# przemo199/ray-tracer-challenge-rs

Measured on AMD Instinct MI355X. Metric: Mray/s (primary+secondary) and ms/frame at 1920x1080, higher is better.
Workload: dtype f32; 1 GPU; three_sphere_scene@1920x1080,depth=5,f32; scene=three_sphere_scene, width=1920, height=1080, max_depth=5, out=real, parallelism=framesx1, rays_per_frame=4147200, stream=side, mode=frames

## Files before the change

profiles/jit/three_sphere_direct.hpp:

```cpp
#pragma once
#include "rtc_internal.hpp"
namespace rtc {
namespace jit {
constexpr int kBegin[7] = {0, 3, 6, 6, 6, 6, 6};
constexpr ShapeRec<float> kShapes[7] = {
    {{__builtin_bit_cast(float, 0x3f800000u), __builtin_bit_cast(float, 0x80000000u), __builtin_bit_cast(float, 0x00000000u), __builtin_bit_cast(float, 0x3f000000u), __builtin_bit_cast(float, 0x80000000u), __builtin_bit_cast(float, 0x3f800000u), __builtin_bit_cast(float, 0x80000000u), __builtin_bit_cast(float, 0xbf800000u), __builtin_bit_cast(float, 0x00000000u), __builtin_bit_cast(float, 0x80000000u), __builtin_bit_cast(float, 0x3f800000u), __builtin_bit_cast(float, 0xbf000000u)}, {__builtin_bit_cast(float, 0xbf000000u), __builtin_bit_cast(float, 0x3f800000u), __builtin_bit_cast(float, 0x3f000000u), __builtin_bit_cast(float, 0x3f805bd1u)}, 3, 1, 1, 774, __builtin_bit_cast(float, 0xff800000u), __builtin_bit_cast(float, 0x7f800000u), {__builtin_bit_cast(float, 0xbf000000u), __builtin_bit_cast(float, 0x3f800000u), __builtin_bit_cast(float, 0x3f000000u), __builtin_bit_cast(float, 0x3f800000u), __builtin_bit_cast(float, 0x00000000u), __builtin_bit_cast(float, 0x00000000u), __builtin_bit_cast(float, 0x00000000u), __builtin_bit_cast(float, 0x00000000u), __builtin_bit_cast(float, 0x00000000u), __builtin_bit_cast(float, 0x00000000u), __builtin_bit_cast(float, 0x00000000u), __builtin_bit_cast(float, 0x00000000u)}},
    {{__builtin_bit_cast(float, 0x40000000u), __builtin_bit_cast(float, 0x80000000u), __builtin_bit_cast(float, 0x00000000u), __builtin_bit_cast(float, 0xc0400000u), __builtin_bit_cast(float, 0x80000000u), __builtin_bit_cast(float, 0x40000000u), __builtin_bit_cast(float, 0x80000000u), __builtin_bit_cast(float, 0xbf800000u), __builtin_bit_cast(float, 0x00000000u), __builtin_bit_cast(float, 0x80000000u), __builtin_bit_cast(float, 0x40000000u), __builtin_bit_cast(float, 0x3f800000u)}, {__builtin_bit_cast(float, 0x3fc00000u), __builtin_bit_cast(float, 0x3f000000u), __builtin_bit_cast(float, 0xbf000000u), __builtin_bit_cast(float, 0x3e807612u)}, 4, 1, 2, 1030, __builtin_bit_cast(float, 0xff800000u), __builtin_bit_cast(float, 0x7f800000u), {__builtin_bit_cast(float, 0x3fc00000u), __builtin_bit_cast(float, 0x3f000000u), __builtin_bit_cast(float, 0xbf000000u), __builtin_bit_cast(float, 0x3e800000u), __builtin_bit_cast(float, 0x00000000u), __builtin_bit_cast(float, 0x00000000u), __builtin_bit_cast(float, 0x00000000u), __builtin_bit_cast(float, 0x00000000u), __builtin_bit_cast(float, 0x00000000u), __builtin_bit_cast(float, 0x00000000u), __builtin_bit_cast(float, 0x00000000u), __builtin_bit_cast(float, 0x00000000u)}},
    {{__builtin_bit_cast(float, 0x4041f07cu), __builtin_bit_cast(float, 0x80000000u), __builtin_bit_cast(float, 0x00000000u), __builtin_bit_cast(float, 0x4091745du), __builtin_bit_cast(float, 0x80000000u), __builtin_bit_cast(float, 0x4041f07cu), __builtin_bit_cast(float, 0x80000000u), __builtin_bit_cast(float, 0xbf800000u), __builtin_bit_cast(float, 0x00000000u), __builtin_bit_cast(float, 0x80000000u), __builtin_bit_cast(float, 0x4041f07cu), __builtin_bit_cast(float, 0x4011745du)}, {__builtin_bit_cast(float, 0xbfc00000u), __builtin_bit_cast(float, 0x3ea8f5c3u), __builtin_bit_cast(float, 0xbf400000u), __builtin_bit_cast(float, 0x3de000b9u)}, 5, 1, 3, 1286, __builtin_bit_cast(float, 0xff800000u), __builtin_bit_cast(float, 0x7f800000u), {__builtin_bit_cast(float, 0xbfc00000u), __builtin_bit_cast(float, 0x3ea8f5c3u), __builtin_bit_cast(float, 0xbf400000u), __builtin_bit_cast(float, 0x3ddf06f7u), __builtin_bit_cast(float, 0x00000000u), __builtin_bit_cast(float, 0x00000000u), __builtin_bit_cast(float, 0x00000000u), __builtin_bit_cast(float, 0x00000000u), __builtin_bit_cast(float, 0x00000000u), __builtin_bit_cast(float, 0x00000000u), __builtin_bit_cast(float, 0x00000000u), __builtin_bit_cast(float, 0x00000000u)}},
    {{__builtin_bit_cast(float, 0x3f800000u), __builtin_bit_cast(float, 0x00000000u), __builtin_bit_cast(float, 0x00000000u), __builtin_bit_cast(float, 0x00000000u), __builtin_bit_cast(float, 0x00000000u), __builtin_bit_cast(float, 0x3f800000u), __builtin_bit_cast(float, 0x00000000u), __builtin_bit_cast(float, 0x00000000u), __builtin_bit_cast(float, 0x00000000u), __builtin_bit_cast(float, 0x00000000u), __builtin_bit_cast(float, 0x3f800000u), __builtin_bit_cast(float, 0x00000000u)}, {__builtin_bit_cast(float, 0x00000000u), __builtin_bit_cast(float, 0x00000000u), __builtin_bit_cast(float, 0x00000000u), __builtin_bit_cast(float, 0xbf800000u)}, 0, 1, 0, 2, __builtin_bit_cast(float, 0xff800000u), __builtin_bit_cast(float, 0x7f800000u), {__builtin_bit_cast(float, 0x00000000u), __builtin_bit_cast(float, 0x00000000u), __builtin_bit_cast(float, 0x00000000u), __builtin_bit_cast(float, 0x00000000u), __builtin_bit_cast(float, 0x00000000u), __builtin_bit_cast(float, 0x00000000u), __builtin_bit_cast(float, 0x00000000u), __builtin_bit_cast(float, 0x00000000u), __builtin_bit_cast(float, 0x00000000u), __builtin_bit_cast(float, 0x00000000u), __builtin_bit_cast(float, 0x00000000u), __builtin_bit_cast(float, 0x00000000u)}},
    {{__builtin_bit_cast(float, 0x3f3b3e17u), __builtin_bit_cast(float, 0x80000000u), __builtin_bit_cast(float, 0x3f2e930eu), __builtin_bit_cast(float, 0xc05a37d2u), __builtin_bit_cast(float, 0xbf2e930eu), __builtin_bit_cast(float, 0xb676812fu), __builtin_bit_cast(float, 0x3f3b3e17u), __builtin_bit_cast(float, 0xc06a0d9du), __builtin_bit_cast(float, 0x36281968u), __builtin_bit_cast(float, 0xbf800000u), __builtin_bit_cast(float, 0xb6344c27u), __builtin_bit_cast(float, 0x37615f30u)}, {__builtin_bit_cast(float, 0x00000000u), __builtin_bit_cast(float, 0x00000000u), __builtin_bit_cast(float, 0x00000000u), __builtin_bit_cast(float, 0xbf800000u)}, 1, 1, 0, 258, __builtin_bit_cast(float, 0xff800000u), __builtin_bit_cast(float, 0x7f800000u), {__builtin_bit_cast(float, 0x00000000u), __builtin_bit_cast(float, 0x00000000u), __builtin_bit_cast(float, 0x00000000u), __builtin_bit_cast(float, 0x00000000u), __builtin_bit_cast(float, 0x00000000u), __builtin_bit_cast(float, 0x00000000u), __builtin_bit_cast(float, 0x00000000u), __builtin_bit_cast(float, 0x00000000u), __builtin_bit_cast(float, 0x00000000u), __builtin_bit_cast(float, 0x00000000u), __builtin_bit_cast(float, 0x00000000u), __builtin_bit_cast(float, 0x00000000u)}},
    {{__builtin_bit_cast(float, 0x3f3b3e17u), __builtin_bit_cast(float, 0x80000000u), __builtin_bit_cast(float, 0xbf2e930eu), __builtin_bit_cast(float, 0x405a37d2u), __builtin_bit_cast(float, 0x3f2e930eu), __builtin_bit_cast(float, 0xb676812fu), __builtin_bit_cast(float, 0x3f3b3e17u), __builtin_bit_cast(float, 0xc06a0d9du), __builtin_bit_cast(float, 0xb6281968u), __builtin_bit_cast(float, 0xbf800000u), __builtin_bit_cast(float, 0xb6344c27u), __builtin_bit_cast(float, 0x37615f30u)}, {__builtin_bit_cast(float, 0x00000000u), __builtin_bit_cast(float, 0x00000000u), __builtin_bit_cast(float, 0x00000000u), __builtin_bit_cast(float, 0xbf800000u)}, 2, 1, 0, 514, __builtin_bit_cast(float, 0xff800000u), __builtin_bit_cast(float, 0x7f800000u), {__builtin_bit_cast(float, 0x00000000u), __builtin_bit_cast(float, 0x00000000u), __builtin_bit_cast(float, 0x00000000u), __builtin_bit_cast(float, 0x00000000u), __builtin_bit_cast(float, 0x00000000u), __builtin_bit_cast(float, 0x00000000u), __builtin_bit_cast(float, 0x00000000u), __builtin_bit_cast(float, 0x00000000u), __builtin_bit_cast(float, 0x00000000u), __builtin_bit_cast(float, 0x00000000u), __builtin_bit_cast(float, 0x00000000u), __builtin_bit_cast(float, 0x00000000u)}},
    {}};
constexpr int kNumClusters = 0;
constexpr float kClusterBall[1][4] = {
    {}};
constexpr int kClusterBegin[1] = {0};
constexpr int kClusterMembers[1] = {0};
constexpr int kNumUnclustered = 6;
constexpr int kUnclustered[6] = {0, 1, 2, 3, 4, 5};
constexpr int kNumLights = 1;
constexpr LightRec<float> kLights[2] = {
    {{__builtin_bit_cast(float, 0xc1200000u), __builtin_bit_cast(float, 0x41200000u), __builtin_bit_cast(float, 0xc1200000u)}, {__builtin_bit_cast(float, 0x3f800000u), __builtin_bit_cast(float, 0x3f800000u), __builtin_bit_cast(float, 0x3f800000u)}},
    {}};
constexpr MaterialRec<float> kMaterials[5] = {
    {{__builtin_bit_cast(float, 0x3f800000u), __builtin_bit_cast(float, 0x3f666666u), __builtin_bit_cast(float, 0x3f666666u)}, __builtin_bit_cast(float, 0x3dcccccdu), __builtin_bit_cast(float, 0x3f666666u), __builtin_bit_cast(float, 0x00000000u), __builtin_bit_cast(float, 0x43480000u), __builtin_bit_cast(float, 0x00000000u), __builtin_bit_cast(float, 0x00000000u), __builtin_bit_cast(float, 0x3f800000u), -1, 1},
    {{__builtin_bit_cast(float, 0x3dcccccdu), __builtin_bit_cast(float, 0x3f800000u), __builtin_bit_cast(float, 0x3f000000u)}, __builtin_bit_cast(float, 0x3dcccccdu), __builtin_bit_cast(float, 0x3f333333u), __builtin_bit_cast(float, 0x3e99999au), __builtin_bit_cast(float, 0x43480000u), __builtin_bit_cast(float, 0x00000000u), __builtin_bit_cast(float, 0x00000000u), __builtin_bit_cast(float, 0x3f800000u), -1, 1},
    {{__builtin_bit_cast(float, 0x3dcccccdu), __builtin_bit_cast(float, 0x3f800000u), __builtin_bit_cast(float, 0x3dcccccdu)}, __builtin_bit_cast(float, 0x3dcccccdu), __builtin_bit_cast(float, 0x3f333333u), __builtin_bit_cast(float, 0x3e99999au), __builtin_bit_cast(float, 0x43480000u), __builtin_bit_cast(float, 0x00000000u), __builtin_bit_cast(float, 0x00000000u), __builtin_bit_cast(float, 0x3f800000u), -1, 1},
    {{__builtin_bit_cast(float, 0x3f800000u), __builtin_bit_cast(float, 0x3f4ccccdu), __builtin_bit_cast(float, 0x3dcccccdu)}, __builtin_bit_cast(float, 0x3dcccccdu), __builtin_bit_cast(float, 0x3f333333u), __builtin_bit_cast(float, 0x3e99999au), __builtin_bit_cast(float, 0x43480000u), __builtin_bit_cast(float, 0x00000000u), __builtin_bit_cast(float, 0x00000000u), __builtin_bit_cast(float, 0x3f800000u), -1, 1},
    {}};
constexpr bool kPatterns = false;
constexpr uint32_t kPatternKinds = 0u;
constexpr bool kTransparent = false;
}
}
```

ray-tracer-challenge-rs_amd/csrc/rtc_host.cpp:

```cpp
#include <hip/hip_runtime.h>

#include <algorithm>
#include <array>
#include <chrono>
#include <cmath>
#include <cstdlib>
#include <cstring>
#include <limits>
#include <memory>
#include <string>
#include <vector>

#include "../../include/rtc.h"
#include "flop_model.hpp"
#include "host_math.hpp"
#include "debug_knobs.hpp"
#include "primary_rect.hpp"
#include "rtc_context.hpp"
#include "rtc_internal.hpp"
#include "shape_identity.hpp"
#include "tri_tree.hpp"
#include "instances.hpp"

namespace rtc {

#define RTC_KERNEL_LAUNCHERS                                                                                          \
    template <typename R>                                                                                             \
    hipError_t launch_trace(const LaunchParams<R>& P, bool pool, bool dup, uint32_t grid, size_t dyn_lds,             \
                            hipStream_t stream);                                                                      \
    template <typename R>                                                                                             \
    hipError_t occupancy(bool pool, bool lds, size_t dyn_lds, int* blocks_per_cu);                                    \
    template <typename R>                                                                                             \
    hipError_t launch_trace_rays(const LaunchParams<R>& P, bool dup, uint32_t grid, size_t dyn_lds, const void* rays, \
                                 void* rgb, void* hits, hipStream_t stream);                                          \
    template <typename R>                                                                                             \
    hipError_t occupancy_rays(bool lds, size_t dyn_lds, int* blocks_per_cu);                                          \
    template <typename R>                                                                                             \
    hipError_t launch_trace_ss(const LaunchParams<R>& P, bool pool, bool dup, uint32_t grid, size_t dyn_lds,          \
                               hipStream_t stream);                                                                   \
    template <typename R>                                                                                             \
    hipError_t occupancy_ss(bool pool, bool lds, size_t dyn_lds, int* blocks_per_cu);
RTC_KERNEL_LAUNCHERS
namespace instanced { RTC_KERNEL_LAUNCHERS }
namespace textured { RTC_KERNEL_LAUNCHERS }
namespace area { RTC_KERNEL_LAUNCHERS }
#undef RTC_KERNEL_LAUNCHERS
namespace sp {
template <typename R>
hipError_t launch_trace(const LaunchParams<R>& P, bool pool, bool dup, uint32_t grid, size_t dyn_lds,
                        hipStream_t stream);
}
constexpr uint32_t kKindsSp = (1u << RT_SHAPE_SPHERE) | (1u << RT_SHAPE_PLANE);

template <typename R>
struct Launchers {
    decltype(&launch_trace<R>) launch_trace;
    decltype(&occupancy<R>) occupancy;
    decltype(&launch_trace_rays<R>) launch_trace_rays;
    decltype(&occupancy_rays<R>) occupancy_rays;
    decltype(&launch_trace_ss<R>) launch_trace_ss;
    decltype(&occupancy_ss<R>) occupancy_ss;
};
#define RTC_BUILD(ns)                                                                                    \
    {ns launch_trace<R>, ns occupancy<R>, ns launch_trace_rays<R>, ns occupancy_rays<R>, ns launch_trace_ss<R>, \
     ns occupancy_ss<R>}
template <typename R>
constexpr Launchers<R> kLaunchers[] = {RTC_BUILD(rtc::), RTC_BUILD(instanced::), RTC_BUILD(textured::), RTC_BUILD(area::)};
#undef RTC_BUILD
template <typename R>
const Launchers<R>& launchers(const rt_context* ctx) {
    return kLaunchers<R>[(uint32_t)ctx->kernel_build];
}

hipError_t launch_order_tiles(uint32_t* cost, uint32_t* order, uint32_t n, uint32_t* n_items, float split_per_cost,
                              uint32_t max_split_log2, float urgent_per_cost, uint32_t graded, uint32_t min_split_log2,
                              hipStream_t stream);
template <typename R>
hipError_t launch_debug_shape(const ShapeRec<R>* shapes, int slot, int kind, uint32_t mode, uint32_t world_space,
                              const double* in, uint32_t n, double* out, hipStream_t stream);

namespace {
thread_local std::string g_error;
}

int set_error(int code, const std::string& msg) {
    g_error = msg;
    return code;
}

void bounding_sphere(const rt_shape_desc& d, double out[4]) {
    out[0] = out[1] = out[2] = 0.0;
    out[3] = -1.0;
    double c[3] = {0.0, 0.0, 0.0}, r = 0.0;
    const double lo = d.minimum, hi = d.maximum;
    switch (d.kind) {
        case RT_SHAPE_SPHERE: r = 1.0; break;
        case RT_SHAPE_CUBE: r = std::sqrt(3.0); break;
        case RT_SHAPE_CYLINDER: {
            if (!std::isfinite(lo) || !std::isfinite(hi) || !(lo <= hi)) return;
            const double half = 0.5 * (hi - lo);
            c[1] = 0.5 * (lo + hi);
            r = std::sqrt(1.0 + half * half);
            break;
        }
        case RT_SHAPE_TRIANGLE: {
            double p[3][3];
            for (int q = 0; q < 3; ++q) {
                p[0][q] = d.vertex_1[q];
                p[1][q] = d.vertex_1[q] + d.edge_1[q];
                p[2][q] = d.vertex_1[q] + d.edge_2[q];
            }
            for (int q = 0; q < 3; ++q) c[q] = (p[0][q] + p[1][q] + p[2][q]) / 3.0;
            for (auto& v : p)
                r = std::max(r, std::sqrt((v[0] - c[0]) * (v[0] - c[0]) + (v[1] - c[1]) * (v[1] - c[1]) +
                                          (v[2] - c[2]) * (v[2] - c[2])));
            break;
        }
        default: return;
    }
    hm::M4 inv;
    for (int i = 0; i < 4; ++i)
        for (int j = 0; j < 4; ++j) inv.m[i][j] = d.inverse[4 * i + j];
    const hm::M4 f = hm::inverse(inv);
    double ftf[3][3] = {}, sigma2 = 0.0;
    for (int i = 0; i < 3; ++i)
        for (int j = 0; j < 3; ++j)
            for (int k = 0; k < 3; ++k) ftf[i][j] += f.m[k][i] * f.m[k][j];
    for (auto& row : ftf) sigma2 = std::max(sigma2, std::fabs(row[0]) + std::fabs(row[1]) + std::fabs(row[2]));
    double wc[3];
    for (int i = 0; i < 3; ++i) wc[i] = f.m[i][0] * c[0] + f.m[i][1] * c[1] + f.m[i][2] * c[2] + f.m[i][3];
    const double wr = r * std::sqrt(sigma2);
    const double scale = std::fabs(wc[0]) + std::fabs(wc[1]) + std::fabs(wc[2]) + wr;
    const double pad = 1e-3 * wr + 1e-4 * scale + 1e-4;
    if (!std::isfinite(wc[0]) || !std::isfinite(wc[1]) || !std::isfinite(wc[2]) || !std::isfinite(wr) ||
        wr + pad > 1e18)
        return;
    for (int i = 0; i < 3; ++i) out[i] = wc[i];
    out[3] = wr + pad;
}

bool similar_sphere(const rt_shape_desc& d, double centre[3], double* r2) {
    if (d.kind != RT_SHAPE_SPHERE) return false;
    hm::M4 inv;
    for (int i = 0; i < 4; ++i)
        for (int j = 0; j < 4; ++j) inv.m[i][j] = d.inverse[4 * i + j];
    if (inv.m[3][0] != 0.0 || inv.m[3][1] != 0.0 || inv.m[3][2] != 0.0 || inv.m[3][3] != 1.0) return false;
    const hm::M4 f = hm::inverse(inv);
    double g[3][3] = {};
    for (int i = 0; i < 3; ++i)
        for (int j = 0; j < 3; ++j)
            for (int k = 0; k < 3; ++k) g[i][j] += f.m[k][i] * f.m[k][j];
    const double s2 = (g[0][0] + g[1][1] + g[2][2]) / 3.0;
    if (!(s2 > 0.0) || !std::isfinite(s2)) return false;
    for (int i = 0; i < 3; ++i)
        for (int j = 0; j < 3; ++j)
            if (!(std::fabs(g[i][j] - (i == j ? s2 : 0.0)) <= 1e-9 * s2)) return false;
    for (int i = 0; i < 3; ++i) {
        centre[i] = f.m[i][3];
        if (!std::isfinite(centre[i])) return false;
    }
    *r2 = s2;
    return true;
}

bool axis_aligned_cube(const rt_shape_desc& d, double face_lo[3], double face_hi[3], double eps[3], double sgn[3]) {
    if (d.kind != RT_SHAPE_CUBE) return false;
    const double* m = d.inverse;
    if (m[12] != 0.0 || m[13] != 0.0 || m[14] != 0.0 || m[15] != 1.0) return false;
    double dmax = 0.0;
// ... 550 lines not shown
    uint64_t n_rays = 0;
    uint32_t depth = 0, out_format = RT_OUT_REAL;
    uint32_t shard_index = 0, shard_count = 1;
    void* out_device = nullptr;
    hipStream_t stream = nullptr;
    uint32_t flags = 0;
    bool image_rows = false;
    uint32_t samples = 0;
    uint32_t out_w = 0, out_h = 0;
};

template <typename R>
void set_instance_params(LaunchParams<R>& P, const DeviceWorld<R>& w) {
    const InstanceCounts& c = w.inst_counts;
    P.n_instances = c.instances;
    P.inst_world_begin = c.instances ? c.world_begin : std::numeric_limits<int32_t>::max();
    P.inst = c.instances ? w.inst.get() : nullptr;
    P.inst_shapes = w.inst_shapes.get();
    P.inst_nodes = w.inst_nodes.get();
    P.inst_pos = w.inst_pos.get();
    P.smooth_plain = w.smooth.plain();
    P.smooth_inst = w.smooth.inst();
    P.uv_plain = w.uv.plain();
    P.uv_inst = w.uv.inst();
    P.texels = w.texels;
    P.textures = w.tex_table;
    P.area = w.n_area ? w.area.get() : nullptr;
    P.n_area = w.n_area;
    P.area_samples = w.area_samples;
    P.area_cull = 1u;
}

template <typename R>
int launch(rt_context* ctx, DeviceWorld<R>& w, const LaunchRequest& q) {
    const rt_camera_desc* cam = q.cam;
    const uint32_t depth = q.depth, flags = q.flags, shard_index = q.shard_index, shard_count = q.shard_count;
    hipStream_t stream = q.stream;
    int rc;
    LaunchParams<R> P{};
    P.image_rows = q.image_rows ? 1u : 0u;
    P.scene = w.scene;
    P.tri_nodes = w.n_tri_nodes ? w.tri_nodes.get() : nullptr;
    P.n_tri_nodes = w.n_tri_nodes;
    P.tri_flat_begin = w.tri_flat_begin;
    set_instance_params(P, w);
    if (!ctx->knobs.area_cull) P.area_cull = 0u;
    if (cam) {
        for (int q = 0; q < 12; ++q) P.cam.inv[q] = (R)cam->inverse[q];
        for (int q = 0; q < 3; ++q) P.cam.origin[q] = (R)cam->origin[q];
        P.cam.half_width = (R)cam->half_width;
        P.cam.half_height = (R)cam->half_height;
        P.cam.pixel_size = (R)cam->pixel_size;
        P.ss_grid = q.samples;
        P.width = q.samples ? q.out_w : cam->width;
        P.height = q.samples ? q.out_h : cam->height;
        P.tiles_x = (P.width + RT_TILE_W - 1) / RT_TILE_W;
        P.tile_rows = tile_rows_for(P.height, shard_count, shard_index);
        P.n_tiles = P.tiles_x * P.tile_rows;
        P.tiles_x_magic = div_magic(P.tiles_x, P.n_tiles);
    } else {
        P.rays = q.d_rays;
        P.n_rays = q.n_rays;
        P.n_tiles = (uint32_t)((q.n_rays + kBlock - 1) / kBlock);
    }
    P.out = q.out_device;
    P.out_format = q.out_format;
    P.shard_index = shard_index;
    P.shard_count = shard_count;
    P.max_depth = depth;
    P.tile_counter = ctx->d_tile_counter.get();
    P.counters = ctx->d_counters.get();
    P.error_flag = ctx->d_error.get();
    if (flags & RT_FLAG_GENERATIONS) P.gen_counts = ctx->d_gen_counts.get();
    if (P.n_tiles == 0) return RT_OK;
    if ((rc = order_after_last(ctx, stream))) return rc;
    LaunchShape ls;
    const bool ss = q.samples != 0;
    rc = plan_launch<R>(ctx, w.scene, depth, P.n_tiles, ls, false, q.samples);
    if (rc) return rc;
    const bool dup = ctx->duplicate_shapes > 0;
    hipFunction_t jf = nullptr;
    if constexpr (sizeof(R) == 4) {
        const uint32_t generic_only =
            RT_FLAG_NO_SHADE | RT_FLAG_NO_TRACE | RT_FLAG_GENERATIONS | (ls.pool ? 0u : RT_FLAG_STAMPS);
        const bool instanced = walked_instances(w), smooth = has_smooth(w);
        const bool tree = w.n_tri_nodes > 0 || instanced || smooth || has_textures(w);
        if (tree && ctx->jit.mode != RT_JIT_OFF && ctx->jit.log.empty())
            ctx->jit.log = has_area(w) ? "no per-scene build: the world has area lights, which the generic kernels sample"
                           : has_textures(w) ? "no per-scene build: the world has textures, which the generic kernels sample"
                           : smooth ? "no per-scene build: the world has smooth triangles, whose normals the generic kernels interpolate"
                           : instanced
                               ? "no per-scene build: the world has mesh instances, which the generic kernels walk"
                               : "no per-scene build: the world has a triangle hierarchy, which the generic kernels walk";
        const bool want = cam && !dup && !tree && !(flags & generic_only) &&
                          (ctx->jit.mode == RT_JIT_SYNC || (ctx->jit.mode >= RT_JIT_AUTO && P.n_tiles >= kJitMinTiles));
        if (want) {
            ++ctx->jit.frames;
            LaunchShape lj = ls;
            if (ctx->knobs.lds_world && !ls.pool && w.scene.kind_begin[kNumKinds] <= kJitRecordsMaxShapes &&
                (rc = plan_launch<R>(ctx, w.scene, depth, P.n_tiles, lj, true, q.samples)))
                return rc;
            int waves = 0;
            if ((rc = jit_function(ctx, lj.pool, lj.world_lds != 0, lj.lds, lj.per_cu, &jf,
                                   (flags & RT_FLAG_NO_SKIPS) != 0, &waves, ss)))
                return rc;
            if (jf && waves > 0 && (rc = plan_pool_for<R>(ctx, jf, lj))) return rc;
            if (jf) ls = lj;
        }
    }
    ctx->jit.used = jf != nullptr;
    P.pool_capacity = ls.cap;
    P.pool_lds_capacity = ls.lcap;
    P.pop_batch = ls.batch;
    if (ls.pool && (rc = check_pixel_range(ctx, depth, sizeof(R) == 4))) return rc;
    P.acc_log2 = acc_shift_f32(ctx->bright_hit, ctx->bright_w, depth);
    if (ls.cap > ls.lcap) {
        const size_t per_block = (size_t)8 * (ls.cap - ls.lcap) * sizeof(R);
        if ((rc = ctx->d_spill.reserve((size_t)ls.grid * per_block))) return rc;
        P.spill = ctx->d_spill.get();
        P.spill_blocks = (uint32_t)(ctx->d_spill.capacity() / per_block);
    }
    P.persistent = ls.sched;
    P.flags = flags;
    P.world_lds = ls.world_lds;
    const bool dynamic = ls.pool;
    if (dynamic) {
        const size_t set = (size_t)kTileQueues * kQueueStride;
        P.tile_counter = ctx->d_tile_counter.get() + (ctx->head_set ? set : 0);
        P.next_tile_counter = ctx->d_tile_counter.get() + (ctx->head_set ? 0 : set);
        if (ls.pool && ctx->knobs.tile_order && cam) {
            if ((rc = plan_tile_order<R>(ctx, ss ? ctx->order_ss : ctx->order, P, cam, depth, ls.grid, stream)))
                return rc;
        }
    }
    if (flags & RT_FLAG_STAMPS) {
        if ((rc = ctx->d_stamps.reserve((size_t)2 * ls.grid))) return rc;
        P.stamps = ctx->d_stamps.get();
        ctx->stamp_count = ls.grid;
        if (ls.pool) {
            const size_t items = (size_t)P.n_tiles << kMaxSplitLog2;
            if ((rc = ctx->d_item_log.reserve(1 + 3 * items))) return rc;
            RT_HIP(hipMemsetAsync(ctx->d_item_log.get(), 0, sizeof(uint64_t), stream));
            P.item_log = ctx->d_item_log.get();
        }
    }
    uint32_t kinds = 0;
    for (int k = 0; k < kNumKinds; ++k)
        if (w.scene.kind_begin[k + 1] > w.scene.kind_begin[k]) kinds |= 1u << k;
    const bool sp = sizeof(R) == 4 && ls.pool && ctx->knobs.kind_variants && (kinds & ~kKindsSp) == 0 && !dup && !ss &&
                    ctx->kernel_build == KernelBuild::plain;
    if (flags & RT_FLAG_FAIL_LAUNCH) return set_error(RT_ERR_HIP, "launch refused (RT_FLAG_FAIL_LAUNCH)");
    if constexpr (sizeof(R) == 4) {
        const size_t ns = ctx->jit.shapes.size();
        if (jf && !ls.pool && cam && !ss && ns <= (size_t)kPrimaryRectSlots && (int)ns == w.scene.kind_begin[kNumKinds] &&
            P.width <= kCullCols * kCullCellW && P.height <= kCullRows * kCullCellH) {
            const uint32_t nc = (P.width + kCullCellW - 1) / kCullCellW, nr = (P.height + kCullCellH - 1) / kCullCellH;
            uint32_t flip_cols[kCullCols + 1] = {}, flip_rows[kCullRows + 1] = {};
            auto outside = [&](const uint32_t r[4], uint32_t b) {
                const bool none = r[0] > r[2] || r[1] > r[3];
                const uint32_t c0 = none ? nc : r[0] / kCullCellW, c1 = none ? nc : r[2] / kCullCellW + 1;
                const uint32_t r0 = none ? nr : r[1] / kCullCellH, r1 = none ? nr : r[3] / kCullCellH + 1;
                flip_cols[0] ^= b, flip_cols[c0] ^= b, flip_cols[c1] ^= b;
                flip_rows[0] ^= b, flip_rows[r0] ^= b, flip_rows[r1] ^= b;
            };
            for (size_t s = 0; s < ns; ++s) {
                uint32_t r[4];
                primary_rect(P.cam, P.width, P.height, ctx->jit.shapes[s].bound, r);
                outside(r, 1u << s);
            }
            const ShadowLayout lay(w.scene.kind_begin, (int)ctx->jit.lights.size());
            if (lay.fits() &&(int)ctx->jit.lights.size() == w.scene.n_lights) {
                for (int p = lay.plane0; p < lay.plane0 + lay.planes; ++p) {
                    const ShapeRec<float>& pl = ctx->jit.shapes[p];
                    const float n[3] = {pl.inv[4], pl.inv[5], pl.inv[6]}, h = -pl.inv[7];
                    uint32_t near[4] = {0, 0, P.width - 1, P.height - 1};
                    for (int l = 0; l < lay.lights; ++l) {
                        const float* lp = ctx->jit.lights[l].position;
                        uint32_t sp[4];
                        shadow_near(P.cam, P.width, P.height, n, h, lp, sp);
                        for (int a = 0; a < 2; ++a) {
                            near[a] = sp[a] > near[a] ? sp[a] : near[a];
                            near[a + 2] = sp[a + 2] < near[a + 2] ? sp[a + 2] : near[a + 2];
                        }
                        for (size_t c = 0; c < ns; ++c) {
                            const int bit = lay.pair_bit(l, p, (int)c);
                            if (bit < 0) continue;
                            if ((int)c == p) {
                                if (shadow_self_clear(P.cam, n, h, lp)) flip_cols[0] ^= 1u << bit;
                                continue;
                            }
                            uint32_t r[4];
                            shadow_rect(P.cam, P.width, P.height, n, h, lp, ctx->jit.shapes[c].bound, r);
                            outside(r, 1u << bit);
                        }
                    }
                    auto blocks = [](uint32_t lo, uint32_t hi, uint32_t cell, uint32_t pixels, uint32_t& b0, uint32_t& b1) {
                        b0 = b1 = 0;
                        if (lo > hi) return;
                        b0 = (lo + cell - 1) / cell;
                        b1 = hi + 1 >= pixels ? (pixels + cell - 1) / cell : (hi + 1) / cell;
                        if (b1 < b0) b1 = b0;
                    };
                    const uint32_t nb = 1u << lay.near_bit(p);
                    uint32_t b0, b1;
                    blocks(near[0], near[2], kCullCellW, P.width, b0, b1);
                    flip_cols[b0] ^= nb, flip_cols[b1] ^= nb;
                    blocks(near[1], near[3], kCullCellH, P.height, b0, b1);
                    flip_rows[b0] ^= nb, flip_rows[b1] ^= nb;
                }
            }
            uint32_t acc = 0;
            for (uint32_t i = 0; i < nc; ++i) P.cull_cols[i] = acc ^= flip_cols[i];
            acc = 0;
            for (uint32_t j = 0; j < nr; ++j) P.cull_rows[j] = acc ^= flip_rows[j];
        }
    }
    if (jf) {
        const ShapeRec<R>* sh = P.scene.shapes;
        const MaterialRec<R>* mt = P.scene.materials;
        const PatternRec<R>* pt = P.scene.patterns;
        const LightRec<R>* lt = P.scene.lights;
        void* args[] = {&P, &sh, &mt, &pt, &lt};
        (void)hipGetLastError();
        RT_HIP(hipModuleLaunchKernel(jf, ls.grid, 1, 1, kBlock, 1, 1, (unsigned)ls.lds, stream, args, nullptr));
    } else if (hipError_t e = ss   ? launchers<R>(ctx).launch_trace_ss(P, ls.pool, dup, ls.grid, ls.lds, stream)
                              : sp ? sp::launch_trace<R>(P, ls.pool, dup, ls.grid, ls.lds, stream)
                                   : launchers<R>(ctx).launch_trace(P, ls.pool, dup, ls.grid, ls.lds, stream);
               e != hipSuccess)
        return set_error(RT_ERR_HIP, std::string("launch of the ") + (ss ? "supersampled " : "") +
                                         (ls.pool ? "pool" : "direct") + " kernel (grid " +
                                         std::to_string(ls.grid) + ", dynamic LDS " + std::to_string(ls.lds) +
                                         " B, pool " + std::to_string(ls.lcap) + "/" + std::to_string(ls.cap) +
                                         " rays in LDS): " + hipGetErrorString(e));
    if (dynamic) ctx->head_set ^= 1;
    ctx->smooth_info.ran_smooth = !jf && has_smooth(w) ? 1u : 0u;
    ctx->texture_info.ran_textured = !jf && has_textures(w) ? 1u : 0u;
    ctx->light_info.ran_area = !jf && has_area(w) ? 1u : 0u;
    return RT_OK;
}

template <typename R>
int ray_blocks_per_cu(rt_context* ctx, bool lds_world, size_t lds, int* per_cu) {
    const int key = 8 + (sizeof(R) == 8 ? 1 : 0) + (lds_world ? 2 : 0);
    if (ctx->occ_lds[key] == lds && ctx->occ_blocks[key] > 0) {
        *per_cu = ctx->occ_blocks[key];
        return RT_OK;
    }
    int api = 0;
    RT_HIP(launchers<R>(ctx).occupancy_rays(lds_world, lds, &api));
    *per_cu = cap_by_lds(api, lds);
    ctx->occ_lds[key] = lds;
    ctx->occ_blocks[key] = *per_cu;
    return RT_OK;
}

template <typename R>
int plan_rays(rt_context* ctx, const DevScene<R>& sc, uint32_t depth, uint32_t n_chunks, LaunchShape& ls) {
    ls.pool = false;
    const size_t wb = world_lds_bytes<R>(sc.kind_begin[kNumKinds], sc.n_materials, sc.n_patterns);
    ls.world_lds = (ctx->knobs.lds_world && wb <= kMaxWorldLds) ? (uint32_t)wb : 0;
    ls.lds = ls.world_lds;
    ls.cap = ray_stack_entries(depth);
    ls.lcap = ls.batch = 0;
    ls.sched = kSchedStatic;
    int per_cu = 0, rc;
    if ((rc = ray_blocks_per_cu<R>(ctx, ls.world_lds != 0, ls.lds, &per_cu))) return rc;
    ls.per_cu = std::max(per_cu, 1);
    const uint64_t resident = (uint64_t)ls.per_cu * (uint64_t)ctx->cu_count;
    ls.grid = (uint32_t)std::max<uint64_t>(1, std::min<uint64_t>(n_chunks, resident));
    ls.grid_tiles = n_chunks;
    return RT_OK;
}

template <typename R>
int launch_rays(rt_context* ctx, DeviceWorld<R>& w, const void* d_rays, uint64_t n, const rt_ray_options* o,
                void* d_rgb, void* d_hits, hipStream_t stream) {
    int rc;
    LaunchParams<R> P{};
    P.scene = w.scene;
    P.tri_nodes = w.n_tri_nodes ? w.tri_nodes.get() : nullptr;
    P.n_tri_nodes = w.n_tri_nodes;
    P.tri_flat_begin = w.tri_flat_begin;
    set_instance_params(P, w);
    if (!ctx->knobs.area_cull) P.area_cull = 0u;
    P.n_rays = n;
    P.n_tiles = (uint32_t)((n + kBlock - 1) / kBlock);
    P.max_depth = o->max_depth;
    P.flags = o->flags;
    P.counters = ctx->d_counters.get();
    P.error_flag = ctx->d_error.get();
    if (o->flags & RT_FLAG_GENERATIONS) P.gen_counts = ctx->d_gen_counts.get();
    if ((rc = order_after_last(ctx, stream))) return rc;
    LaunchShape ls;
    if ((rc = plan_rays<R>(ctx, w.scene, o->max_depth, P.n_tiles, ls))) return rc;
    P.pool_capacity = ls.cap;
    P.persistent = ls.sched;
    P.world_lds = ls.world_lds;
    if (ls.cap) {
        const size_t per_block = ray_stack_word(1, ls.cap, 0, 0) * sizeof(R);
        if ((rc = ctx->d_spill.reserve((size_t)ls.grid * per_block))) return rc;
        P.spill = ctx->d_spill.get();
        P.spill_blocks = (uint32_t)std::min<size_t>(ctx->d_spill.capacity() / per_block, 0xFFFFFFFFu);
    }
    ctx->jit.used = false;
    if (o->flags & RT_FLAG_FAIL_LAUNCH) return set_error(RT_ERR_HIP, "launch refused (RT_FLAG_FAIL_LAUNCH)");
    if (hipError_t e = launchers<R>(ctx).launch_trace_rays(P, ctx->duplicate_shapes > 0, ls.grid, ls.lds, d_rays, d_rgb,
                                                           d_hits, stream);
        e != hipSuccess)
// ... 1563 lines not shown
```

ray-tracer-challenge-rs_amd/csrc/rtc_internal.hpp:

```cpp
#pragma once

#include <cstdint>
#ifndef __HIPCC_RTC__
#include <string>
#endif

#include "../../include/rtc.h"

#if defined(__HIP__)
#define RTC_HD __host__ __device__
#else
#define RTC_HD
#endif

namespace rtc {

#ifndef __HIPCC_RTC__
int set_error(int code, const std::string& msg);
#endif

RTC_HD inline uint32_t shard_tile_rows(uint32_t height, uint32_t shards, uint32_t shard) {
    const uint32_t trows = (height + RT_TILE_H - 1) / RT_TILE_H;
    return trows > shard ? (trows - shard + shards - 1) / shards : 0;
}
RTC_HD inline uint32_t shard_image_row(uint32_t strip_row, uint32_t shards, uint32_t shard) {
    return ((strip_row / RT_TILE_H) * shards + shard) * RT_TILE_H + strip_row % RT_TILE_H;
}
RTC_HD inline void shard_of_image_row(uint32_t y, uint32_t shards, uint32_t* shard, uint32_t* strip_row) {
    const uint32_t trow = y / RT_TILE_H;
    *shard = trow % shards;
    *strip_row = (trow / shards) * RT_TILE_H + y % RT_TILE_H;
}

constexpr int kBlock = 256;
constexpr int kWaves = kBlock / 64;
constexpr int kTileSlots = 1;
constexpr uint32_t kPoolBatch = kBlock;
constexpr int kTilePixels = RT_TILE_W * RT_TILE_H;
static_assert(kTilePixels == kBlock, "one pixel per thread per tile");
constexpr int kNumKinds = 6;
constexpr int kNumCounters = 8;
constexpr int kGenSlots = RT_MAX_SUPPORTED_DEPTH + 1;
constexpr int kCounterShards = 256;
constexpr int kTileQueues = 8;
constexpr int kQueueStride = 32;
constexpr uint32_t kItemTileMask = 0xFFFFFu;
constexpr uint32_t kItemPartShift = 20, kItemSplitShift = 26, kItemPartMask = 63u, kItemSplitMask = 7u;
constexpr uint32_t kItemPrioShift = 29;
constexpr uint32_t kMaxSplitLog2 = 6;
constexpr int kOrderBuilds = 8;
constexpr uint32_t kNoItem = 0xFFFFFFFFu;

struct WorkItem {
    uint32_t tile, part, split_log2, prio;
};
RTC_HD inline WorkItem decode_item(uint32_t item, bool packed) {
    if (!packed) return {item, 0u, 0u, 0u};
    return {item & kItemTileMask, (item >> kItemPartShift) & kItemPartMask, (item >> kItemSplitShift) & kItemSplitMask,
            (item >> kItemPrioShift) & 3u};
}
RTC_HD inline uint32_t encode_item(uint32_t tile, uint32_t part, uint32_t split_log2, uint32_t prio) {
    return tile | part << kItemPartShift | split_log2 << kItemSplitShift | prio << kItemPrioShift;
}
RTC_HD inline bool item_seeds(uint32_t tid, const WorkItem& w) { return (tid >> (8u - w.split_log2)) == w.part; }

RTC_HD inline uint64_t spill_word(uint32_t block, uint32_t spill_cap, uint32_t slot, uint32_t lds_cap) {
    return ((uint64_t)block * spill_cap + (slot - lds_cap)) * 8u;
}

RTC_HD inline uint32_t pool_capacity_ss(uint32_t depth, uint32_t batch, uint32_t grid) {
    (void)grid;
    return (uint32_t)kBlock + depth * batch;
}

RTC_HD inline uint32_t ray_stack_entries(uint32_t max_depth) { return max_depth ? max_depth + 1u : 0u; }
RTC_HD inline uint64_t ray_stack_word(uint32_t block, uint32_t entries, uint32_t e, uint32_t tid) {
    return (((uint64_t)block * entries + e) * 256u + tid) * 8u;
}
constexpr uint64_t kMaxRayBatch = 1ull << 31;

constexpr int32_t kErrPoolOverflow = 1;
constexpr int32_t kErrPoolSpin = 2;
constexpr int32_t kErrBoundsSlot = 4;
constexpr int32_t kErrBoundsSpill = 8;
constexpr int32_t kErrBoundsTile = 16;
constexpr int32_t kErrBoundsOut = 32;
constexpr int32_t kErrPeerTimeout = 64;
constexpr int32_t kErrBitsAll[] = {kErrPoolOverflow, kErrPoolSpin, kErrBoundsSlot, kErrBoundsSpill,
                                   kErrBoundsTile, kErrBoundsOut, kErrPeerTimeout};
#ifndef __HIPCC_RTC__
inline std::string device_error_text(int32_t err) {
    std::string m;
    auto add = [&](int32_t bit, const char* what) {
        if (err & bit) m += (m.empty() ? "" : "; ") + std::string(what);
    };
    add(kErrPoolOverflow, "device ray pool overflow: a child beyond the LIFO bound");
    add(kErrPoolSpin, "device ray pool: a lock's spin bound ran out (a starved wave, not an overflow)");
    add(kErrBoundsSlot, "bounds check: pool slot outside the LIFO bound");
    add(kErrBoundsSpill, "bounds check: spill region outside the spill buffer");
    add(kErrBoundsTile, "bounds check: work item tile outside the launch");
    add(kErrBoundsOut, "bounds check: output index outside the canvas");
    add(kErrPeerTimeout, "peer canvas: a shard's flag (or the owner's release) did not arrive within the timeout");
    const int32_t unknown = err & ~(kErrPoolOverflow | kErrPoolSpin | kErrBoundsSlot | kErrBoundsSpill |
                                    kErrBoundsTile | kErrBoundsOut | kErrPeerTimeout);
    if (unknown) m += (m.empty() ? "" : "; ") + std::string("device error bits ") + std::to_string(unknown);
    return m;
}
#endif

constexpr uint64_t kCanvasFlagAlign = 256;
RTC_HD inline uint32_t div_magic(uint32_t d, uint32_t n) {
    if (d < 2 || (uint64_t)n * d >= (1ull << 32)) return 0;
    return (uint32_t)(((1ull << 32) + d - 1) / d);
}
RTC_HD inline uint32_t div_by(uint32_t t, uint32_t d, uint32_t magic) {
    return magic ? (uint32_t)(((uint64_t)t * magic) >> 32) : t / d;
}

RTC_HD inline uint64_t canvas_flag_offset(uint64_t image_bytes) {
    return (image_bytes + kCanvasFlagAlign - 1) / kCanvasFlagAlign * kCanvasFlagAlign;
}
constexpr uint32_t kSchedGrid = 0;
constexpr uint32_t kSchedDynamic = 1;
constexpr uint32_t kSchedStatic = 2;
constexpr size_t kMaxWorldLds = 16 * 1024;

constexpr double kAccScale = 281474976710656.0;
constexpr double kAccInvScale = 1.0 / 281474976710656.0;
template <bool B, typename T, typename F>
struct Choose {
    using type = T;
};
template <typename T, typename F>
struct Choose<false, T, F> {
    using type = F;
};
#ifndef RTC_ACC_I64
template <typename R>
using PoolAcc = typename Choose<sizeof(R) == 4, int32_t, long long>::type;
#else
template <typename R>
using PoolAcc = long long;
#endif
constexpr uint32_t kAccLog2Min = 8, kAccLog2Max = 28;
#ifndef RTC_POOL_META32
using PoolMeta = uint16_t;
#else
using PoolMeta = uint32_t;
#endif
static_assert(RT_MAX_SUPPORTED_DEPTH < 32, "remaining must fit the pool meta's 8 high bits");

constexpr int32_t kShapeClosed = 1;
constexpr int32_t kShapeClassEnd = 2;
constexpr int32_t kShapeSimilar = 4;
constexpr int32_t kShapeAxisAligned = 8;
constexpr int32_t kShapeSmooth = 16;
constexpr int kSmoothReals = 9;
constexpr int32_t kShapeUV = 32;
constexpr int kUVReals = 6;
struct alignas(16) TexRec {
    uint64_t offset;
    uint32_t width, height;
};
static_assert(sizeof(TexRec) == 16);
constexpr int kShapeClassShift = 8;

template <typename R>
struct alignas(16) ShapeRec {
    R inv[12];
    R bound[4];
    int32_t world_index;
    int32_t casts_shadow;
    int32_t material;
    int32_t flags;
    R ymin, ymax;
    R tri[12];
};

template <typename R>
struct alignas(16) MaterialRec {
    R color[3];
    R ambient, diffuse, specular, shininess;
    R reflectiveness, transparency, refractive_index;
    int32_t pattern;
    int32_t casts_shadow;
};

template <typename R>
struct alignas(16) PatternRec {
    R color_a[3];
    R color_b[3];
    R inv[12];
    int32_t kind;
    int32_t sub_a, sub_b;
    int32_t pad;
};

template <typename R>
constexpr size_t world_lds_bytes(size_t ns, size_t nm, size_t np) {
    return ns * sizeof(ShapeRec<R>) + nm * sizeof(MaterialRec<R>) + np * sizeof(PatternRec<R>) +
           (ns + 3) / 4 * 16;
}
static_assert(sizeof(ShapeRec<float>) % 16 == 0 && sizeof(ShapeRec<double>) % 16 == 0);
static_assert(sizeof(MaterialRec<float>) % 16 == 0 && sizeof(MaterialRec<double>) % 16 == 0);
static_assert(sizeof(PatternRec<float>) % 16 == 0 && sizeof(PatternRec<double>) % 16 == 0);

template <typename R>
struct alignas(16) LightRec {
    R position[3];
    R intensity[3];
};

template <typename R>
struct alignas(16) AreaLightRec {
    R corner[3];
    R uvec[3];
    R vvec[3];
    R intensity[3];
    uint32_t usteps, vsteps, jitter, seed;
};
static_assert(sizeof(AreaLightRec<float>) == 64 && sizeof(AreaLightRec<double>) == 112);

template <typename R>
struct CameraRec {
    R inv[12];
    R origin[3];
    R half_width, half_height, pixel_size;
};

template <typename R>
struct alignas(16) TriNode {
    R ball[4];
    int32_t skip, first, count, pad;
};
static_assert(sizeof(TriNode<float>) == 32 && sizeof(TriNode<double>) == 48);

template <typename R>
struct alignas(16) InstRec {
    R inv[12];
    R ball[4];
    int32_t world_base;
    int32_t casts_shadow;
    int32_t material;
    int32_t n_triangles;
    int32_t node_begin, n_nodes;
    int32_t rec_begin;
    int32_t rec_flat;
    int32_t rec_end;
    int32_t pos_begin;
    int32_t expanded;
    int32_t pad;
};
static_assert(sizeof(InstRec<float>) % 16 == 0 && sizeof(InstRec<double>) % 16 == 0);

template <typename Base>
RTC_HD inline int instance_of_world(Base&& base, int n, int w) {
    int lo = 0, hi = n;
    while (hi - lo > 1) {
        const int mid = (lo + hi) >> 1;
        if (base(mid) <= w) lo = mid;
        else hi = mid;
    }
    return lo;
}

template <typename R>
struct DevScene {
    const ShapeRec<R>* shapes;
    const MaterialRec<R>* materials;
    const PatternRec<R>* patterns;
    const LightRec<R>* lights;
    const int32_t* world_slot;
    const ShapeRec<R>* lshapes;
    const MaterialRec<R>* lmats;
    const PatternRec<R>* lpats;
    const int32_t* lworld_slot;
    int32_t kind_begin[kNumKinds + 1];
    int32_t n_materials, n_patterns;
    int32_t n_lights;
    int32_t any_secondary;
    int32_t no_skips;
};

constexpr int kPrimaryRectSlots = 8;
constexpr uint32_t kCullCellW = 16, kCullCellH = 4;
constexpr uint32_t kCullCols = 128, kCullRows = 512;

constexpr int kShadowRectSlots = 6;
constexpr int kShadowBit0 = kPrimaryRectSlots, kShadowBits = 32 - kPrimaryRectSlots;
struct ShadowLayout {
    int planes, casters, lights, plane0;
    constexpr ShadowLayout(const int32_t* kb, int n_lights)
        : planes(kb[RT_SHAPE_PLANE + 1] - kb[RT_SHAPE_PLANE]), casters(kb[kNumKinds] - planes), lights(n_lights),
          plane0(kb[RT_SHAPE_PLANE]) {}
    constexpr bool fits() const {
        return planes > 0 && lights > 0 && planes + casters <= kShadowRectSlots &&
               planes + lights * planes * (casters + 1) <= kShadowBits;
    }
    constexpr bool is_plane(int slot) const { return slot >= plane0 && slot < plane0 + planes; }
    constexpr int near_bit(int slot) const { return kShadowBit0 + (slot - plane0); }
    constexpr int pair_bit(int light, int slot, int c) const {
        if (is_plane(c) && c != slot) return -1;
        const int rank = c == slot ? casters : (c < plane0 ? c : c - planes);
        return kShadowBit0 + planes + (light * planes + (slot - plane0)) * (casters + 1) + rank;
    }
};

template <typename R>
struct LaunchParams {
    DevScene<R> scene;
    CameraRec<R> cam;
    const double* rays;
    uint64_t n_rays;
    void* out;
    uint32_t out_format;
    uint32_t width, height;
    uint32_t tiles_x;
    uint32_t tile_rows;
    uint32_t image_rows;
    uint32_t shard_index, shard_count;
    uint32_t n_tiles;
    uint32_t max_depth;
    uint32_t pool_capacity;
    uint32_t pool_lds_capacity;
    uint32_t pop_batch;
    uint32_t acc_log2;
    uint32_t persistent;
    uint32_t flags;
    uint32_t world_lds;
    void* spill;
    uint32_t spill_blocks;
    uint32_t tiles_x_magic;
    unsigned long long* stamps;
    unsigned long long* item_log;
    unsigned long long* tile_counter;
    unsigned long long* next_tile_counter;
    const uint32_t* tile_order;
    const uint32_t* item_count;
    uint32_t* tile_cost;
    unsigned long long* counters;
    unsigned long long* gen_counts;
    int32_t* error_flag;
    uint32_t cull_cols[kCullCols];
    uint32_t cull_rows[kCullRows];
    uint32_t ss_grid;
    uint32_t n_tri_nodes;
    const TriNode<R>* tri_nodes;
    uint32_t tri_flat_begin;
    uint32_t n_instances;
    int32_t inst_world_begin;
    const InstRec<R>* inst;
    const ShapeRec<R>* inst_shapes;
    const TriNode<R>* inst_nodes;
    const int32_t* inst_pos;
    const R* smooth_plain;
    const R* smooth_inst;
    const R* uv_plain;
    const R* uv_inst;
    const uint32_t* texels;
    const TexRec* textures;
    const AreaLightRec<R>* area;
    uint32_t n_area;
    uint32_t area_samples;
    uint32_t area_cull;
};

}
```

ray-tracer-challenge-rs_amd/csrc/rtc_jit.cpp:

```cpp
#include <hip/hip_runtime.h>
#include <hip/hiprtc.h>

#include <algorithm>
#include <array>
#include <atomic>
#include <cmath>
#include <cerrno>
#include <chrono>
#include <condition_variable>
#include <cstdio>
#include <cstdlib>
#include <cstring>
#include <map>
#include <memory>
#include <mutex>
#include <string>
#include <thread>
#include <vector>

#include <dirent.h>
#include <dlfcn.h>
#include <fcntl.h>
#include <spawn.h>
#include <sys/stat.h>
#include <sys/wait.h>
#include <unistd.h>

#include "debug_knobs.hpp"
#include "jit_options.hpp"
#include "rtc_context.hpp"
#include "rtc_jit_cache.hpp"
#include "rtc_jit_sources.inc"

extern char** environ;

namespace rtc {

struct CodeBuild {
    std::atomic<int> state{0};
    jitfile::CodeObject co;
    std::string log;
    double ms = 0;
    bool from_disk = false;
};

namespace {

using jitfile::fnv;

std::string hexf(float v) {
    uint32_t b;
    std::memcpy(&b, &v, 4);
    char buf[48];
    std::snprintf(buf, sizeof buf, "__builtin_bit_cast(float, 0x%08xu)", b);
    return buf;
}

template <size_t N>
std::string floats(const float (&a)[N]) {
    std::string s = "{";
    for (size_t i = 0; i < N; ++i) s += (i ? ", " : "") + hexf(a[i]);
    return s + "}";
}
std::string ball4(const float* a) {
    std::string s = "{";
    for (size_t i = 0; i < 4; ++i) s += (i ? ", " : "") + hexf(a[i]);
    return s + "}";
}

constexpr int kClusterMinShapes = 6;
struct Clusters {
    std::vector<std::array<float, 4>> ball;
    std::vector<int> begin, members, unclustered;
};
Clusters make_clusters(const std::vector<ShapeRec<float>>& sh) {
    Clusters c;
    std::vector<int> bounded;
    for (int i = 0; i < (int)sh.size(); ++i) {
        const float r2 = sh[i].bound[3];
        if (std::isfinite(r2) && r2 >= 0.0f) bounded.push_back(i);
        else c.unclustered.push_back(i);
    }
    std::string knob;
    const char* e = debug_knob("jit_clusters", &knob) ? knob.c_str() : nullptr;
    const int n = (int)bounded.size();
    auto flat = [&]() {
        c.unclustered.insert(c.unclustered.end(), bounded.begin(), bounded.end());
        std::sort(c.unclustered.begin(), c.unclustered.end());
        c.ball.clear();
        c.members.clear();
        c.begin = {0};
        return c;
    };
    const int forced = e ? std::atoi(e) : 0;
    if ((n < kClusterMinShapes && !(forced >= 1 && n >= 2)) || (e && !std::strcmp(e, "0"))) return flat();
    using P3 = std::array<double, 3>;
    auto ctr = [&](int i) { return P3{sh[i].bound[0], sh[i].bound[1], sh[i].bound[2]}; };
    auto rad = [&](int i) { return std::sqrt((double)sh[i].bound[3]); };
    auto d2 = [](const P3& a, const P3& b) {
        return (a[0] - b[0]) * (a[0] - b[0]) + (a[1] - b[1]) * (a[1] - b[1]) + (a[2] - b[2]) * (a[2] - b[2]);
    };
    struct Cl {
        P3 cent;
        double r;
        std::vector<int> m;
    };
    auto kmeans = [&](int k) {
        std::vector<P3> cent{ctr(bounded[0])};
        while ((int)cent.size() < k) {
            int far = bounded[0];
            double best = -1.0;
            for (int i : bounded) {
                double m = 1e300;
                for (const auto& q : cent) m = std::min(m, d2(ctr(i), q));
                if (m > best) best = m, far = i;
            }
            cent.push_back(ctr(far));
        }
        std::vector<int> lab(n, 0);
        for (int it = 0; it < 32; ++it) {
            for (int j = 0; j < n; ++j) {
                double m = 1e300;
                for (int q = 0; q < k; ++q)
                    if (const double v = d2(ctr(bounded[j]), cent[q]); v < m) m = v, lab[j] = q;
            }
            for (int q = 0; q < k; ++q) {
                P3 sum{0, 0, 0};
                int cnt = 0;
                for (int j = 0; j < n; ++j)
                    if (lab[j] == q) {
                        const P3 a = ctr(bounded[j]);
                        for (int t = 0; t < 3; ++t) sum[t] += a[t];
                        ++cnt;
                    }
                if (cnt) cent[q] = {sum[0] / cnt, sum[1] / cnt, sum[2] / cnt};
            }
        }
        std::vector<Cl> out;
        for (int q = 0; q < k; ++q) {
            Cl cl{cent[q], 0.0, {}};
            for (int j = 0; j < n; ++j)
                if (lab[j] == q) {
                    cl.m.push_back(bounded[j]);
                    cl.r = std::max(cl.r, std::sqrt(d2(ctr(bounded[j]), cent[q])) + rad(bounded[j]));
                }
            if (!cl.m.empty()) out.push_back(cl);
        }
        return out;
    };
    P3 mid{0, 0, 0};
    for (int i : bounded)
        for (int t = 0; t < 3; ++t) mid[t] += ctr(i)[t] / n;
    double world = 0.0;
    for (int i : bounded) world = std::max(world, std::sqrt(d2(ctr(i), mid)) + rad(i));
    constexpr double kMemberWeight = 2.0;
    std::string rknob;
    const char* rf = debug_knob("jit_cluster_refine", &rknob) ? rknob.c_str() : nullptr;
    const bool refine = !(rf && !std::strcmp(rf, "0")) && n <= 64;
    auto ball_of = [&](Cl& q) {
        q.cent = {0, 0, 0};
        for (int i : q.m)
            for (int t = 0; t < 3; ++t) q.cent[t] += ctr(i)[t] / (double)q.m.size();
        q.r = 0.0;
        for (int i : q.m) q.r = std::max(q.r, std::sqrt(d2(ctr(i), q.cent)) + rad(i));
    };
    auto term = [&](const Cl& q) { return (double)q.m.size() * q.r * q.r; };
    auto refine_clusters = [&](std::vector<Cl>& cl) {
        for (int guard = 0; guard < 256; ++guard) {
            double best_gain = 1e-9 * world * world;
            int ba = -1, bs = -1, bb = -1;
            for (int a = 0; a < (int)cl.size(); ++a) {
                if (cl[a].m.size() < 2) continue;
                for (int si = 0; si < (int)cl[a].m.size(); ++si)
                    for (int b = 0; b < (int)cl.size(); ++b) {
                        if (b == a) continue;
                        Cl na = cl[a], nb = cl[b];
                        na.m.erase(na.m.begin() + si);
                        nb.m.push_back(cl[a].m[si]);
                        ball_of(na);
                        ball_of(nb);
                        const double gain = term(cl[a]) + term(cl[b]) - term(na) - term(nb);
                        if (gain > best_gain) best_gain = gain, ba = a, bs = si, bb = b;
                    }
            }
            if (ba < 0) break;
            cl[bb].m.push_back(cl[ba].m[bs]);
            cl[ba].m.erase(cl[ba].m.begin() + bs);
            ball_of(cl[ba]);
            ball_of(cl[bb]);
        }
        for (Cl& q : cl) std::sort(q.m.begin(), q.m.end());
    };
    std::vector<Cl> best;
    double best_cost = 0.8 * kMemberWeight * n;
    for (int k = forced == 1 ? 1 : 2; k <= std::min(8, n - 1); ++k) {
        if (forced >= 1 && k != std::min(forced, n - 1)) continue;
        std::vector<Cl> cl = kmeans(k);
        if (refine) refine_clusters(cl);
        double cost = (double)cl.size();
        for (const Cl& q : cl) cost += kMemberWeight * (double)q.m.size() * std::min(1.0, (q.r / world) * (q.r / world));
        if (cost < best_cost || forced >= 1) best_cost = cost, best = std::move(cl);
    }
    if (best.empty()) return flat();
    c.begin.push_back(0);
    for (const Cl& q : best) {
        c.members.insert(c.members.end(), q.m.begin(), q.m.end());
        const double pad = 1e-4 * (q.r + std::fabs(q.cent[0]) + std::fabs(q.cent[1]) + std::fabs(q.cent[2])) + 1e-4;
        c.ball.push_back({(float)q.cent[0], (float)q.cent[1], (float)q.cent[2], (float)((q.r + pad) * (q.r + pad))});
        c.begin.push_back((int)c.members.size());
    }
    return c;
}

std::string scene_header(const std::vector<ShapeRec<float>>& sh, const int32_t begin[kNumKinds + 1],
                         const std::vector<LightRec<float>>& lights, const std::vector<MaterialRec<float>>& mats,
                         bool patterns, uint32_t pattern_kinds, bool transparent) {
    std::string s = "#pragma once\n#include \"rtc_internal.hpp\"\nnamespace rtc {\nnamespace jit {\n";
    s += "constexpr int kBegin[" + std::to_string(kNumKinds + 1) + "] = {";
    for (int k = 0; k <= kNumKinds; ++k) s += (k ? ", " : "") + std::to_string(begin[k]);
    s += "};\nconstexpr ShapeRec<float> kShapes[" + std::to_string(sh.size() + 1) + "] = {\n";
    for (const ShapeRec<float>& r : sh) {
        s += "    {" + floats(r.inv) + ", " + floats(r.bound) + ", " + std::to_string(r.world_index) + ", " +
             std::to_string(r.casts_shadow) + ", " + std::to_string(r.material) + ", " + std::to_string(r.flags) +
             ", " + hexf(r.ymin) + ", " + hexf(r.ymax) + ", " + floats(r.tri) + "},\n";
    }
    s += "    {}};\n";
    const Clusters cl = make_clusters(sh);
    auto ints = [](const std::vector<int>& v) {
        std::string o = "{";
        for (size_t i = 0; i < v.size(); ++i) o += (i ? ", " : "") + std::to_string(v[i]);
        return o + (v.empty() ? "0}" : "}");
    };
    s += "constexpr int kNumClusters = " + std::to_string(cl.ball.size()) + ";\n";
    s += "constexpr float kClusterBall[" + std::to_string(cl.ball.size() + 1) + "][4] = {\n";
    for (const auto& b : cl.ball) s += "    " + ball4(b.data()) + ",\n";
    s += "    {}};\n";
    s += "constexpr int kClusterBegin[" + std::to_string(cl.begin.size()) + "] = " + ints(cl.begin) + ";\n";
    s += "constexpr int kClusterMembers[" + std::to_string(std::max<size_t>(1, cl.members.size())) + "] = " +
         ints(cl.members) + ";\n";
    s += "constexpr int kNumUnclustered = " + std::to_string(cl.unclustered.size()) + ";\n";
    s += "constexpr int kUnclustered[" + std::to_string(std::max<size_t>(1, cl.unclustered.size())) + "] = " +
         ints(cl.unclustered) + ";\n";
    s += "constexpr int kNumLights = " + std::to_string(lights.size()) + ";\n";
    s += "constexpr LightRec<float> kLights[" + std::to_string(lights.size() + 1) + "] = {\n";
    for (const LightRec<float>& l : lights) s += "    {" + floats(l.position) + ", " + floats(l.intensity) + "},\n";
    s += "    {}};\n";
    s += "constexpr MaterialRec<float> kMaterials[" + std::to_string(mats.size() + 1) + "] = {\n";
    for (const MaterialRec<float>& m : mats) {
        s += "    {" + floats(m.color) + ", " + hexf(m.ambient) + ", " + hexf(m.diffuse) + ", " + hexf(m.specular) + ", " +
             hexf(m.shininess) + ", " + hexf(m.reflectiveness) + ", " + hexf(m.transparency) + ", " +
             hexf(m.refractive_index) + ", " + std::to_string(m.pattern) + ", " + std::to_string(m.casts_shadow) + "},\n";
    }
    s += "    {}};\n";
    s += std::string("constexpr bool kPatterns = ") + (patterns ? "true" : "false") + ";\n";
    s += "constexpr uint32_t kPatternKinds = " + std::to_string(pattern_kinds) + "u;\n";
    s += std::string("constexpr bool kTransparent = ") + (transparent ? "true" : "false") + ";\n";
    s += "}  // namespace jit\n}  // namespace rtc\n";
    return s;
}

const char* kernel_name(bool pool, bool lds, bool ss) {
    if (ss) {
        if (pool) return lds ? "rtc::trace_pool_ss<float, true, false>" : "rtc::trace_pool_ss<float, false, false>";
        return lds ? "rtc::trace_direct_ss<float, true>" : "rtc::trace_direct_ss<float, false>";
    }
    if (pool) return lds ? "rtc::trace_pool<float, true, false>" : "rtc::trace_pool<float, false, false>";
    return lds ? "rtc::trace_direct<float, true>" : "rtc::trace_direct<float, false>";
}

uint64_t file_identity(const char* path, uint64_t h) {
    struct stat st;
    if (!path || ::stat(path, &st) != 0) return fnv("?", 1, h);
    h = fnv(path, std::strlen(path) + 1, h);
    const int64_t v[2] = {(int64_t)st.st_size, (int64_t)st.st_mtime};
    return fnv(v, sizeof v, h);
}

std::string librtc_dir() {
    Dl_info self{};
    if (!dladdr(reinterpret_cast<void*>(&scene_header), &self) || !self.dli_fname) return ".";
    std::string p(self.dli_fname);
    const size_t slash = p.find_last_of('/');
    return slash == std::string::npos ? "." : p.substr(0, slash);
}

uint64_t toolchain_identity() {
    static const uint64_t id = [] {
        uint64_t h = 1469598103934665603ull;
        int v[4] = {};
        hiprtcVersion(&v[0], &v[1]);
        (void)hipRuntimeGetVersion(&v[2]);
        (void)hipDriverGetVersion(&v[3]);
        h = fnv(v, sizeof v, h);
        Dl_info self{}, rtcc{};
        if (dladdr(reinterpret_cast<void*>(&scene_header), &self)) h = file_identity(self.dli_fname, h);
        if (dladdr(reinterpret_cast<void*>(&hiprtcCompileProgram), &rtcc) && rtcc.dli_fname) {
            h = file_identity(rtcc.dli_fname, h);
            std::string dir(rtcc.dli_fname);
            dir = dir.substr(0, dir.find_last_of('/') + 1);
            if (DIR* d = ::opendir(dir.empty() ? "." : dir.c_str())) {
                std::vector<std::string> names;
                while (dirent* e = ::readdir(d))
                    if (std::strstr(e->d_name, "amd_comgr")) names.push_back(e->d_name);
                ::closedir(d);
                std::sort(names.begin(), names.end());
                for (const std::string& n : names) h = file_identity((dir + n).c_str(), h);
            }
        }
        return h;
    }();
    return id;
}

std::vector<std::string> build_defines() {
    std::vector<std::string> out;
    const std::string all(kBuildExtra);
    for (size_t p = 0; p < all.size();) {
        size_t q = all.find_first_of(" \t\n", p);
        if (q == std::string::npos) q = all.size();
        const std::string tok = all.substr(p, q - p);
        if (tok.size() > 2 && tok[0] == '-' && (tok[1] == 'D' || tok[1] == 'U')) out.push_back(tok);
        p = q + 1;
    }
    return out;
}

jitfile::Request make_request(const std::string& scene, const char* name, const std::string& arch, uint64_t* key,
                              bool no_skips, int pool_waves) {
    jitfile::Request rq;
    rq.name = name;
    rq.main_src = std::string("#define RTC_JIT 1\n#include \"rtc_jit_scene.hpp\"\n") + kSrcKernels;
    rq.headers = {{"rtc_jit_scene.hpp", scene}, {"rtc_internal.hpp", kSrcInternal}, {"../../include/rtc.h", kSrcRtcH}};
    rq.opts = {"--offload-arch=" + arch, "-O3", "-std=c++20", "-ffp-contract=off", "-fno-slp-vectorize", "-mllvm",
               "-disable-machine-licm"};
    static const std::vector<std::string> defines = build_defines();
    rq.opts.insert(rq.opts.end(), defines.begin(), defines.end());
    const auto kind = jit_kind_defines(std::strstr(name, "pool") != nullptr, no_skips, pool_waves);
    rq.opts.insert(rq.opts.end(), kind.begin(), kind.end());
    if (std::string all; debug_knob("jit_flags", &all)) {
        for (size_t p = 0; p < all.size();) {
            size_t q = all.find_first_of(" ,", p);
            if (q == std::string::npos) q = all.size();
            if (q > p) rq.opts.push_back(all.substr(p, q - p));
            p = q + 1;
        }
    }
    uint64_t k = fnv(rq.main_src.data(), rq.main_src.size());
    for (const auto& h : rq.headers) k = fnv(h.second.data(), h.second.size() + 1, fnv(h.first.data(), h.first.size() + 1, k));
    for (const std::string& o : rq.opts) k = fnv(o.data(), o.size() + 1, k);
    k = fnv(rq.name.data(), rq.name.size() + 1, k);
    const uint64_t tool = toolchain_identity();
    *key = fnv(&tool, sizeof tool, k);
    return rq;
}

std::string cache_dir() {
    const char* e = std::getenv("RTC_JIT_CACHE");
    if (e) return (!*e || !std::strcmp(e, "0")) ? std::string() : std::string(e);
    if (const char* x = std::getenv("XDG_CACHE_HOME"); x && *x) return std::string(x) + "/rtc_jit";
    if (const char* h = std::getenv("HOME"); h && *h) return std::string(h) + "/.cache/rtc_jit";
    return std::string();
}

std::string cache_path(const std::string& dir, uint64_t key) {
    char buf[32];
    std::snprintf(buf, sizeof buf, "/%016llx.co", (unsigned long long)key);
    return dir + buf;
}

std::string temp_path(const char* suffix) {
    static std::atomic<unsigned> seq{0};
    const char* t = std::getenv("TMPDIR");
    return std::string(t && *t ? t : "/tmp") + "/rtcjit-" + std::to_string((long long)::getpid()) + "-" +
           std::to_string(seq++) + suffix;
}

std::mutex& g_mu = *new std::mutex;
std::condition_variable& g_cv = *new std::condition_variable;
auto& g_code = *new std::map<std::pair<uint64_t, int>, std::shared_ptr<CodeBuild>>;
auto& g_fn = *new std::map<std::pair<uint64_t, int>, std::pair<hipModule_t, hipFunction_t>>;

void finish(const std::shared_ptr<CodeBuild>& b, bool ok, std::string log) {
    {
        std::lock_guard<std::mutex> lk(g_mu);
        b->log = std::move(log);
        b->state.store(ok ? 1 : 2, std::memory_order_release);
    }
    g_cv.notify_all();
}

void await_child(std::shared_ptr<CodeBuild> b, pid_t pid, int fd, std::string out, bool temp_out,
                 std::chrono::steady_clock::time_point t0) {
    std::string log;
    char buf[4096];
    for (;;) {
        const ssize_t n = ::read(fd, buf, sizeof buf);
        if (n > 0) {
            if (log.size() < (1u << 20)) log.append(buf, (size_t)n);
        } else if (n < 0 && errno == EINTR) {
            continue;
        } else {
            break;
        }
    }
    ::close(fd);
    int status = 0;
    pid_t w;
    do {
        w = ::waitpid(pid, &status, 0);
    } while (w < 0 && errno == EINTR);
    const bool exited_ok = w < 0 ? true : (WIFEXITED(status) && WEXITSTATUS(status) == 0);
    const bool ok = exited_ok && jitfile::read_code(out, b->co);
    if (temp_out) std::remove(out.c_str());
    b->ms = std::chrono::duration<double, std::milli>(std::chrono::steady_clock::now() - t0).count();
    if (!ok && log.empty()) log = "rtc_jitc failed (status " + std::to_string(status) + ")";
    finish(b, ok, ok ? std::string() : "per-scene build failed: " + log);
}

void start_build(const std::shared_ptr<CodeBuild>& b, const jitfile::Request& rq, uint64_t key, bool sync) {
    const auto t0 = std::chrono::steady_clock::now();
    const std::string dir = cache_dir();
    const std::string path = dir.empty() ? std::string() : cache_path(dir, key);
    if (!path.empty() && jitfile::read_code(path, b->co)) {
        b->from_disk = true;
        b->ms = std::chrono::duration<double, std::milli>(std::chrono::steady_clock::now() - t0).count();
        finish(b, true, std::string());
        return;
    }
    const char* env_helper = std::getenv("RTC_JITC");
    const std::string helper = env_helper && *env_helper ? env_helper : librtc_dir() + "/rtc_jitc";
    if (::access(helper.c_str(), X_OK) != 0) {
        finish(b, false, "per-scene build: compiler " + helper + " not found (the generic kernel is used)");
        return;
    }
    const std::string req = temp_path(".req");
    const bool temp_out = path.empty();
    const std::string out = temp_out ? temp_path(".co") : path;
    if (!jitfile::write_request(req, rq)) {
        finish(b, false, "per-scene build: cannot write " + req);
        return;
    }
    int fds[2];
    if (::pipe2(fds, O_CLOEXEC) != 0) {
        std::remove(req.c_str());
        finish(b, false, std::string("per-scene build: pipe: ") + std::strerror(errno));
        return;
    }
    posix_spawn_file_actions_t fa;
    posix_spawn_file_actions_init(&fa);
    posix_spawn_file_actions_adddup2(&fa, fds[1], 1);
    posix_spawn_file_actions_adddup2(&fa, fds[1], 2);
    std::vector<char*> argv = {const_cast<char*>(helper.c_str()), const_cast<char*>(req.c_str()),
                               const_cast<char*>(out.c_str()), nullptr};
    pid_t pid = 0;
    const int e = posix_spawn(&pid, helper.c_str(), &fa, nullptr, argv.data(), environ);
    posix_spawn_file_actions_destroy(&fa);
    ::close(fds[1]);
    if (e != 0) {
        ::close(fds[0]);
        std::remove(req.c_str());
        finish(b, false, std::string("per-scene build: cannot start ") + helper + ": " + std::strerror(e));
        return;
    }
    if (sync) {
        await_child(b, pid, fds[0], out, temp_out, t0);
        return;
    }
    try {
        std::thread(await_child, b, pid, fds[0], out, temp_out, t0).detach();
    } catch (const std::exception&) {
        await_child(b, pid, fds[0], out, temp_out, t0);
    }
}

}

const std::string& device_arch(rt_context* ctx) {
    if (ctx->jit.arch.empty()) {
        hipDeviceProp_t prop;
        if (hipSetDevice(ctx->device) == hipSuccess && hipGetDeviceProperties(&prop, ctx->device) == hipSuccess) {
            const std::string a(prop.gcnArchName);
            ctx->jit.arch = a.empty() ? std::string("gfx950") : a.substr(0, a.find(':'));
        } else {
            ctx->jit.arch = "gfx950";
        }
    }
    return ctx->jit.arch;
}

constexpr int kPool7ScratchMax = 40;
constexpr int kPoolSsScratchMax = 80;

namespace {
int jit_variant(rt_context* ctx, int variant, bool pool, bool lds, size_t dyn_lds, int static_blocks,
                hipFunction_t* fn, bool no_skips, int pool_waves, int scratch_max, bool start_only = false,
                bool ss = false) {
    *fn = nullptr;
    if (ctx->jit.fn[variant]) {
        *fn = ctx->jit.fn[variant];
        return RT_OK;
    }
    if (ctx->jit.rejected[variant]) return RT_OK;
    const bool sync = ctx->jit.mode == RT_JIT_SYNC;
    std::shared_ptr<CodeBuild>& b = ctx->jit.build[variant];
    if (!b) {
        uint64_t table = fnv(ctx->jit.begin, sizeof ctx->jit.begin,
                             fnv(ctx->jit.shapes.data(), ctx->jit.shapes.size() * sizeof(ShapeRec<float>)));
        table = fnv(ctx->jit.lights.data(), ctx->jit.lights.size() * sizeof(LightRec<float>), table);
        table = fnv(ctx->jit.materials.data(), ctx->jit.materials.size() * sizeof(MaterialRec<float>), table);
        const uint32_t traits[3] = {ctx->jit.patterns, ctx->jit.pattern_kinds, ctx->jit.transparent};
        table = fnv(traits, sizeof traits, table);
        const std::string& arch = device_arch(ctx);
        table = fnv(arch.data(), arch.size() + 1, table);
        const uint32_t start_at = ctx->jit.mode == RT_JIT_AUTO ? 2 : 1;
        bool start = false;
        {
            std::lock_guard<std::mutex> lk(g_mu);
            auto it = g_code.find({table, variant});
            if (it != g_code.end()) {
                b = it->second;
            } else if (sync || ctx->jit.frames >= start_at) {
                b = std::make_shared<CodeBuild>();
                g_code[{table, variant}] = b;
                start = true;
            }
        }
        if (!b) return RT_OK;
        if (start) {
            ctx->jit.owner[variant] = true;
            uint64_t key = 0;
            const jitfile::Request rq =
                make_request(scene_header(ctx->jit.shapes, ctx->jit.begin, ctx->jit.lights, ctx->jit.materials,
                                          ctx->jit.patterns,
                                          ctx->jit.pattern_kinds, ctx->jit.transparent),
                             kernel_name(pool, lds, ss), device_arch(ctx), &key, no_skips, pool_waves);
            start_build(b, rq, key, sync && !start_only);
        }
    }
    if (start_only) return RT_OK;
    if (sync) {
        std::unique_lock<std::mutex> lk(g_mu);
        g_cv.wait(lk, [&] { return b->state.load() != 0; });
    }
    const int state = b->state.load(std::memory_order_acquire);
    if (state == 0) return RT_OK;
    if (ctx->jit.owner[variant]) {
        ctx->jit.compile_ms += b->ms;
        if (b->from_disk) ++ctx->jit.cache_hits;
        ctx->jit.owner[variant] = false;
    }
    const bool optional = (variant & (8 | 16)) != 0;
    if (state == 2) {
        (optional ? ctx->jit.rejected[variant] : ctx->jit.failed) = true;
        ctx->jit.log = b->log;
        return RT_OK;
    }
    std::pair<hipModule_t, hipFunction_t> mf{};
    {
        std::lock_guard<std::mutex> lk(g_mu);
        auto it = g_fn.find({(uint64_t)(uintptr_t)b.get(), ctx->device});
        if (it != g_fn.end()) mf = it->second;
    }
    if (!mf.second) {
        RT_HIP(hipSetDevice(ctx->device));
        hipError_t e = hipModuleLoadData(&mf.first, b->co.code.data());
        if (e == hipSuccess) {
            e = hipModuleGetFunction(&mf.second, mf.first, b->co.lowered.c_str());
            if (e != hipSuccess) {
                (void)hipModuleUnload(mf.first);
                mf = {};
            }
        }
        if (e != hipSuccess) {
            (void)hipGetLastError();
            (optional ? ctx->jit.rejected[variant] : ctx->jit.failed) = true;
            ctx->jit.log = std::string("per-scene kernel not loaded (") + ctx->jit.arch + "): " + hipGetErrorString(e);
            return RT_OK;
        }
        std::lock_guard<std::mutex> lk(g_mu);
        auto ins = g_fn.emplace(std::make_pair((uint64_t)(uintptr_t)b.get(), ctx->device), mf);
        if (!ins.second) {
            (void)hipModuleUnload(mf.first);
            mf = ins.first->second;
        }
    }
    int blocks = 0, scratch = 0;
    RT_HIP(hipModuleOccupancyMaxActiveBlocksPerMultiprocessor(&blocks, mf.second, kBlock, dyn_lds));
    RT_HIP(hipFuncGetAttribute(&scratch, HIP_FUNC_ATTRIBUTE_LOCAL_SIZE_BYTES, mf.second));
    if (std::string v; ss && pool && debug_knob("jit_ss_scratch", &v)) scratch_max = std::atoi(v.c_str());
    if (blocks < static_blocks || scratch > (pool ? scratch_max : 0)) {
        ctx->jit.rejected[variant] = true;
        ctx->jit.log = std::string("per-scene ") + (ss ? "supersampled " : "") + (pool ? "pool" : "direct") +
                       " kernel not used: " +
                       std::to_string(blocks) + " workgroups/CU (generic " + std::to_string(static_blocks) + "), " +
                       std::to_string(scratch) + " B/lane of scratch";
        return RT_OK;
    }
    ctx->jit.fn[variant] = mf.second;
    *fn = mf.second;
    return RT_OK;
}
}

int jit_function(rt_context* ctx, bool pool, bool lds, size_t dyn_lds, int static_blocks, hipFunction_t* fn,
                 bool no_skips, int* pool_waves, bool ss) {
    *fn = nullptr;
    if (pool_waves) *pool_waves = 0;
    if (ctx->jit.failed || ctx->jit.shapes.empty()) return RT_OK;
    const int variant = (ss ? 16 : 0) + (no_skips ? 4 : 0) + (pool ? 2 : 0) + (lds ? 1 : 0);
    if (!pool) return jit_variant(ctx, variant, pool, lds, dyn_lds, static_blocks, fn, no_skips, 0, 0, false, ss);
    if (ss)
        return jit_variant(ctx, variant, pool, lds, dyn_lds, static_blocks, fn, no_skips, 0, kPoolSsScratchMax, false,
                           ss);
    int rc = jit_variant(ctx, variant, pool, lds, dyn_lds, static_blocks, fn, no_skips, 0, 16, true);
    if (rc) return rc;
    rc = jit_variant(ctx, variant + 8, pool, lds, dyn_lds, static_blocks, fn, no_skips, 7, kPool7ScratchMax);
    if (rc || ctx->jit.failed) return rc;
    if (*fn) {
        if (pool_waves) *pool_waves = 7;
        return RT_OK;
    }
    return jit_variant(ctx, variant, pool, lds, dyn_lds, static_blocks, fn, no_skips, 0, 16);
}

int jit_wait(rt_context* ctx, double timeout_ms, int* pending) {
    const auto deadline = std::chrono::steady_clock::now() +
                          std::chrono::microseconds((int64_t)(timeout_ms < 0 ? 3.6e12 : timeout_ms * 1e3));
    auto left = [ctx] {
        int n = 0;
        for (const auto& b : ctx->jit.build) n += b && b->state.load() == 0;
        return n;
    };
    std::unique_lock<std::mutex> lk(g_mu);
    g_cv.wait_until(lk, deadline, [&] { return left() == 0; });
    if (pending) *pending = left();
    return RT_OK;
}

}
```

ray-tracer-challenge-rs_amd/csrc/rtc_kernels.hip:

```cpp
#ifndef RTC_INSTANCES
#define RTC_INSTANCES 0
#endif
#ifndef RTC_AREA_LIGHTS
#define RTC_AREA_LIGHTS 0
#endif
#ifndef RTC_TEXTURES
#define RTC_TEXTURES 0
#endif
#if defined(RTC_VARIANT) && !RTC_INSTANCES
#define RTC_POOL_ONLY 1
#endif
#ifndef __HIPCC_RTC__
#include <hip/hip_runtime.h>

#include <cstdint>
#endif

#include "rtc_internal.hpp"

namespace rtc {
#ifdef RTC_VARIANT
namespace RTC_VARIANT {
#endif

// ... 474 lines not shown
            }
        } else {
            first = n ? (int)kernarg_params<R>().tri_flat_begin : sc.kind_begin[RT_SHAPE_TRIANGLE];
            end = sc.kind_begin[RT_SHAPE_TRIANGLE + 1];
        }
        ++i;
        for (int j = first; j < end; ++j) {
            const ShapeRec<R> s = ld_uniform(&sc.shapes[j]);
            f(s, j);
        }
    }
#if RTC_INSTANCES
    if (P.n_instances) for_instances<R, kHalfLine>(o, d, dd, f);
#endif
#endif
}

template <typename R, bool kHalfLine, typename F>
__device__ inline void for_all_kinds(const DevScene<R>& sc, V3<R> o, V3<R> d, R dd, F&& f) {
    for_kind_if<R, RT_SHAPE_SPHERE>(sc, [&](const ShapeRec<R>& s, int i) { f.template operator()<RT_SHAPE_SPHERE>(s, i); });
    for_kind_if<R, RT_SHAPE_PLANE>(sc, [&](const ShapeRec<R>& s, int i) { f.template operator()<RT_SHAPE_PLANE>(s, i); });
    for_kind_if<R, RT_SHAPE_CUBE>(sc, [&](const ShapeRec<R>& s, int i) { f.template operator()<RT_SHAPE_CUBE>(s, i); });
    for_kind_if<R, RT_SHAPE_CYLINDER>(sc,
                                   [&](const ShapeRec<R>& s, int i) { f.template operator()<RT_SHAPE_CYLINDER>(s, i); });
    for_kind_if<R, RT_SHAPE_CONE>(sc, [&](const ShapeRec<R>& s, int i) { f.template operator()<RT_SHAPE_CONE>(s, i); });
    if constexpr ((RTC_KINDS >> RT_SHAPE_TRIANGLE) & 1)
        for_triangles<R, kHalfLine>(sc, o, d, dd,
                                    [&](const ShapeRec<R>& s, int i) { f.template operator()<RT_SHAPE_TRIANGLE>(s, i); });
}

template <typename R, bool kNearest, typename F>
__device__ inline void sphere_world(const ShapeRec<R>& s, V3<R> o, V3<R> d, R dd, R rdd, F&& emit) {
    const V3<R> oc = {s.tri[0] - o.x, s.tri[1] - o.y, s.tri[2] - o.z};
    const R tc = dot(d, oc);
    const V3<R> c = cross(d, oc);
    const R disc = s.tri[3] * dd - dot(c, c);
    const bool v = !(disc < (R)0);
    const R root = Real<R>::sqrt(disc);
    const R t1 = (tc - root) * rdd, t2 = (tc + root) * rdd;
    if constexpr (kNearest) {
        emit(sel(t1 >= (R)0, t1, t2), v);
    } else {
        emit(t1, v);
        emit(t2, v);
    }
}
template <typename R, bool kNearest, typename F>
__device__ inline void cube_world(const ShapeRec<R>& s, V3<R> o, V3<R> d, V3<R> rd, F&& emit) {
    using T = Real<R>;
    auto axis = [&](int i, R org, R dir, R rdir, R& lo, R& hi) {
        const bool steep = T::fabs(dir) >= s.tri[6 + i];
        const R r = sel(steep, rdir, s.tri[9 + i] * T::kMax);
        const R l = (s.tri[i] - org) * r, h = (s.tri[3 + i] - org) * r;
        const bool swap = l > h;
        lo = sel(swap, h, l);
        hi = sel(swap, l, h);
    };
    R xn, xx, yn, yx, zn, zx;
    axis(0, o.x, d.x, rd.x, xn, xx);
    axis(1, o.y, d.y, rd.y, yn, yx);
    axis(2, o.z, d.z, rd.z, zn, zx);
    const R tmin = T::fmax(T::fmax(T::fmax(-T::kMax, xn), yn), zn);
    const R tmax = T::fmin(T::fmin(T::fmin(T::kMax, xx), yx), zx);
    const bool v = (tmin < tmax) & (tmax > (R)0);
    if constexpr (kNearest) {
        emit(sel(tmin >= (R)0, tmin, tmax), v);
    } else {
        emit(tmin, v);
        emit(tmax, v);
    }
}
template <typename R, int K>
__device__ inline bool world_cube(const ShapeRec<R>& s) {
    if constexpr (sizeof(R) == 4 && K == RT_SHAPE_CUBE) return (s.flags & kShapeAxisAligned) != 0;
    return false;
}
template <typename R>
__device__ inline V3<R> recip3(V3<R> d) {
    if constexpr (sizeof(R) == 4)
        return {__builtin_amdgcn_rcpf(d.x), __builtin_amdgcn_rcpf(d.y), __builtin_amdgcn_rcpf(d.z)};
    else return {(R)1 / d.x, (R)1 / d.y, (R)1 / d.z};
}
template <typename R, int K>
__device__ inline bool world_sphere(const ShapeRec<R>& s) {
    if constexpr (sizeof(R) == 4 && K == RT_SHAPE_SPHERE) return (s.flags & kShapeSimilar) != 0;
    return false;
}
template <typename R>
__device__ inline R recip(R x) {
    if constexpr (sizeof(R) == 4) return __builtin_amdgcn_rcpf(x);
    else return (R)1 / x;
}

__device__ inline bool wave_any(bool p) { return __builtin_amdgcn_ballot_w64(p) != 0; }

template <typename R, bool kHalfLine>
__device__ inline bool wave_ball_may_hit(R cx, R cy, R cz, R r2, V3<R> o, V3<R> d, R dd) {
    const V3<R> oc = {cx - o.x, cy - o.y, cz - o.z};
    constexpr R kKeep = sizeof(R) == 4 ? (R)(1 - 1e-5) : (R)(1 - 1e-12);
    const R tc = dot(oc, d), oo = dot(oc, oc);
    if constexpr (!kHalfLine) return wave_any(Real<R>::madd(oo, kKeep, -r2) * dd <= tc * tc);
    const unsigned long long front = __builtin_amdgcn_ballot_w64(tc >= (R)0) | __builtin_amdgcn_ballot_w64(oo <= r2);
    return (front & __builtin_amdgcn_ballot_w64(Real<R>::madd(oo, kKeep, -r2) * dd <= tc * tc)) != 0;
}

#ifndef RTC_SHADOW_LIGHT_CULL
#define RTC_SHADOW_LIGHT_CULL 1
#endif
template <typename R>
__device__ inline bool wave_ball_may_hit_from(R cx, R cy, R cz, R r2, V3<R> l, V3<R> tl, R tt) {
    constexpr R kKeep = sizeof(R) == 4 ? (R)(1 - 1e-5) : (R)(1 - 1e-12);
    const V3<R> cl = {cx - l.x, cy - l.y, cz - l.z};
    const R k = Real<R>::madd(dot(cl, cl), kKeep, -r2);
    if (!(k > (R)0)) return true;
    const R tc = dot(cl, tl);
    return (__builtin_amdgcn_ballot_w64(tc <= (R)0) & __builtin_amdgcn_ballot_w64(k * tt <= tc * tc)) != 0;
}

template <typename R, int K>
__device__ inline bool wave_may_hit(const ShapeRec<R>& s, V3<R> o, V3<R> d, R dd) {
    if constexpr (K == RT_SHAPE_PLANE) return true;
    const R r2 = s.bound[3];
    if constexpr (K != RT_SHAPE_SPHERE && K != RT_SHAPE_CUBE)
        if (!(r2 >= (R)0)) return true;
    return wave_ball_may_hit<R, true>(s.bound[0], s.bound[1], s.bound[2], r2, o, d, dd);
}

#ifndef RTC_WALK_CULL_MIN
#define RTC_WALK_CULL_MIN 4
#endif
template <typename R, int K>
__device__ inline bool wave_line_may_hit(const ShapeRec<R>& s, V3<R> o, V3<R> d, R dd) {
    if constexpr (K == RT_SHAPE_PLANE) return true;
    const R r2 = s.bound[3];
    if constexpr (K != RT_SHAPE_SPHERE && K != RT_SHAPE_CUBE)
        if (!(r2 >= (R)0)) return true;
    return wave_ball_may_hit<R, false>(s.bound[0], s.bound[1], s.bound[2], r2, o, d, dd);
}

#ifndef RTC_JIT_FENCE_EVERY
#define RTC_JIT_FENCE_EVERY 1
#endif
#ifndef RTC_JIT_FENCE_MIN_SHAPES
#define RTC_JIT_FENCE_MIN_SHAPES 0
#endif
template <typename R>
__device__ inline void jit_fence(V3<R>& o, V3<R>& d, int slot = 0) {
#if defined(RTC_JIT) && !defined(RTC_JIT_NO_FENCE)
    if constexpr (sizeof(R) == 4 && jit::kBegin[kNumKinds] >= RTC_JIT_FENCE_MIN_SHAPES)
        if (slot % RTC_JIT_FENCE_EVERY == 0)
            asm volatile("" : "+v"(o.x), "+v"(o.y), "+v"(o.z), "+v"(d.x), "+v"(d.y), "+v"(d.z));
#endif
}

#ifdef RTC_JIT
constexpr int jit_kind_of(int slot) {
    int k = 0;
    while (k < kNumKinds - 1 && slot >= jit::kBegin[k + 1]) ++k;
    return k;
}
template <int M, typename F>
__device__ inline void jit_unclustered(F&& f) {
    if constexpr (M < jit::kNumUnclustered) {
        constexpr int slot = jit::kUnclustered[M];
        f.template operator()<jit_kind_of(slot)>(jit::kShapes[slot], slot);
        jit_unclustered<M + 1>(f);
    }
}
template <int C, int M, typename F>
__device__ inline void jit_members(F&& f) {
    if constexpr (M < jit::kClusterBegin[C + 1]) {
        constexpr int slot = jit::kClusterMembers[M];
        f.template operator()<jit_kind_of(slot)>(jit::kShapes[slot], slot);
        jit_members<C, M + 1>(f);
    }
}
template <int C>
constexpr bool jit_cluster_convex() {
    for (int m = jit::kClusterBegin[C]; m < jit::kClusterBegin[C + 1]; ++m) {
        const int k = jit_kind_of(jit::kClusterMembers[m]);
        if (k != RT_SHAPE_SPHERE && k != RT_SHAPE_CUBE) return false;
    }
    return true;
}
template <bool kHalfLine, bool kBall, int C, typename F, typename S>
__device__ inline void jit_clusters(V3<float>& o, V3<float>& d, float dd, F&& f, S&& skip) {
    if constexpr (C < jit::kNumClusters) {
        jit_fence(o, d);
        if (!skip(jit::kClusterBall[C][0], jit::kClusterBall[C][1], jit::kClusterBall[C][2], jit::kClusterBall[C][3],
                  jit_cluster_convex<C>()) &&
            (!kBall || wave_ball_may_hit<float, kHalfLine>(jit::kClusterBall[C][0], jit::kClusterBall[C][1],
                                                           jit::kClusterBall[C][2], jit::kClusterBall[C][3], o, d, dd)))
            jit_members<C, jit::kClusterBegin[C]>(f);
        jit_clusters<kHalfLine, kBall, C + 1>(o, d, dd, f, skip);
    }
}
#endif
struct NoSkip {
    template <typename... A>
    __device__ bool operator()(A...) const {
        return false;
    }
};
template <typename R, bool kHalfLine, bool kBall = true, typename F, typename S = NoSkip>
__device__ inline void for_all_culled(const DevScene<R>& sc, V3<R>& o, V3<R>& d, R dd, F&& f, S&& skip = S{}) {
#ifdef RTC_JIT
    if constexpr (sizeof(R) == 4 && jit::kNumClusters > 0) {
        jit_unclustered<0>(f);
        jit_clusters<kHalfLine, kBall, 0>(o, d, dd, f, skip);
        return;
    }
#endif
    (void)skip;
    for_all_kinds<R, kHalfLine>(sc, o, d, dd, f);
}

template <typename R>
struct Hit {
    R t;
    int slot;
    int world;
    int kind;
};

#ifndef RTC_VALU_KEYS
#define RTC_VALU_KEYS 1
#endif
template <typename R>
struct Nearest {
    static constexpr bool kKeys = sizeof(R) == 4 && RTC_VALU_KEYS;
    static_assert(!(kJitRecords && sizeof(R) == 4) || kKeys, "per-scene records need RTC_VALU_KEYS");
    R t = Real<R>::kInf;
    int w = __INT_MAX__;
    unsigned long long key = 0x7F8000007FFFFFFFull;
    __device__ inline void offer(R te, bool v, int we) {
        if constexpr (kKeys) {
            const float tv = v ? te : -1.0f;
            const unsigned long long k = ((unsigned long long)__float_as_uint(tv + 0.0f) << 32) | (uint32_t)we;
            const bool better = k < key;
            key = better ? k : key;
            t = better ? te : t;
        } else {
            const bool better = v & (te >= (R)0) & ((te < t) | ((te == t) & (we < w)));
            t = sel(better, te, t);
            w = better ? we : w;
        }
    }
    __device__ inline Hit<R> hit(const DevScene<R>& sc) const {
        const int hw = kKeys ? (int)(uint32_t)key : w;
        Hit<R> h{t, -1, hw, -1};
        if constexpr (kJitRecords && kKeys) {
            if (hw != __INT_MAX__) {
                h.world = hw >> 8;
                h.slot = hw & 0xFF;
            }
            return h;
        }
#if !defined(RTC_JIT) && RTC_INSTANCES
        if (hw != __INT_MAX__ && hw >= kernarg_params<R>().inst_world_begin) {
            const LaunchParams<R>& P = kernarg_params<R>();
            const InstRec<R>* const inst = P.inst;
            const int k = instance_of_world([&](int i) { return inst[i].world_base; }, (int)P.n_instances, hw);
            const int32_t e = P.inst_pos[inst[k].pos_begin + (hw - inst[k].world_base)];
            const bool plain = inst[k].expanded != 0;
            h.slot = plain ? (int)((uint32_t)e & 0xFFFFFFu) : e;
            h.kind = plain ? (int)((uint32_t)e >> 24) : (RT_SHAPE_TRIANGLE | ((k + 1) << 8));
            return h;
        }
#endif
        if (hw != __INT_MAX__) {
            const uint32_t ws = (uint32_t)sc.lworld_slot[hw];
            h.slot = (int)(ws & 0xFFFFFFu);
            h.kind = (int)(ws >> 24);
        }
        return h;
    }
};

#ifndef RTC_CUBE_EXIT_PATH
#define RTC_CUBE_EXIT_PATH 1
#endif
template <typename R>
__device__ inline bool jit_cube_holds_light(const ShapeRec<R>& s) {
#if defined(RTC_JIT) && RTC_CUBE_EXIT_PATH
    if constexpr (sizeof(R) == 4) {
        bool any = false;
        for (int i = 0; i < jit::kNumLights; ++i) {
            const V3<R> p = xform_point(s.inv, V3<R>{jit::kLights[i].position[0], jit::kLights[i].position[1],
                                                     jit::kLights[i].position[2]});
            constexpr R kIn = (R)(1 - 1e-4);
            any |= Real<R>::fabs(p.x) < kIn && Real<R>::fabs(p.y) < kIn && Real<R>::fabs(p.z) < kIn;
        }
        return any;
    }
#endif
    (void)s;
    return false;
}

template <typename R>
__device__ inline bool skips_on(const DevScene<R>& sc) {
#ifdef RTC_NO_SKIPS
    (void)sc;
    return false;
#else
#ifdef RTC_JIT
    if constexpr (sizeof(R) == 4) return true;
#endif
    return !sc.no_skips;
#endif
}

#ifndef RTC_PRIMARY_RECTS
#define RTC_PRIMARY_RECTS 1
#endif
struct NoBlock {
    static constexpr bool kOn = false;
    __device__ bool misses(int) const { return false; }
};
struct PixelBlock {
    static constexpr bool kOn = true;
    uint32_t miss;
    __device__ inline bool misses(int slot) const { return (miss >> slot) & 1u; }
};

template <typename R, typename B = NoBlock>
__device__ inline Hit<R> closest_hit(const DevScene<R>& sc, V3<R> o, V3<R> d, B blk = B{}) {
    Nearest<R> best;
#if defined(RTC_JIT) && !defined(RTC_NO_SKIPS) && RTC_PRIMARY_RECTS
    constexpr bool kRects = B::kOn && sizeof(R) == 4 && jit::kBegin[kNumKinds] <= kPrimaryRectSlots;
    constexpr bool kLazy = kRects && jit::kNumClusters == 0;
#else
    constexpr bool kRects = false, kLazy = false;
#endif
    R dd0 = (R)0, rdd0 = (R)0;
    V3<R> rd0 = {(R)0, (R)0, (R)0};
    if constexpr (!kLazy) {
        dd0 = dot(d, d);
        rdd0 = recip(dd0);
        rd0 = recip3(d);
    }
    for_all_culled<R, true>(sc, o, d, dd0, [&]<int K>(const ShapeRec<R>& s, int slot) {
        jit_fence(o, d, slot);
        if constexpr (kRects && K != RT_SHAPE_PLANE)
            if (blk.misses(slot)) return;
        const R dd = kLazy ? dot(d, d) : dd0;
        if (!wave_may_hit<R, K>(s, o, d, dd)) return;
        const int w = kJitRecords && sizeof(R) == 4 ? (s.world_index << 8) | slot : s.world_index;
        if (world_sphere<R, K>(s)) {
            const R rdd = kLazy ? recip(dd) : rdd0;
            sphere_world<R, true>(s, o, d, dd, rdd, [&](R t, bool v) { best.offer(t, v, w); });
            return;
        }
        if (world_cube<R, K>(s)) {
            const V3<R> rd = kLazy ? recip3(d) : rd0;
            cube_world<R, true>(s, o, d, rd, [&](R t, bool v) { best.offer(t, v, w); });
            return;
        }
        const V3<R> lo = xform_point(s.inv, o);
        const V3<R> ld = xform_vector(s.inv, d);
        if (K == RT_SHAPE_PLANE && skips_on(sc)) {
            if (!wave_any(!(lo.y * ld.y > (R)0))) return;
        }
        if constexpr (K == RT_SHAPE_CUBE && sizeof(R) == 4) {
            if (jit_cube_holds_light(s) && skips_on(sc) &&
                !wave_any(!(Real<R>::fabs(lo.x) < (R)1 && Real<R>::fabs(lo.y) < (R)1 && Real<R>::fabs(lo.z) < (R)1))) {
                using T = Real<R>;
                auto hi = [](auto org, auto dir) {
                    const bool steep = T::fabs(dir) >= T::kEps;
                    const R r = sel(steep, __builtin_amdgcn_rcpf(dir), T::kMax);
                    return sel(r > (R)0, (R)1 - org, (R)-1 - org) * r;
                };
                const R tmax = T::fmin(T::fmin(T::fmin(T::kMax, hi(lo.x, ld.x)), hi(lo.y, ld.y)), hi(lo.z, ld.z));
                best.offer(tmax, tmax > (R)0, w);
                return;
            }
        }
        entries<R, K, true>(s, lo, ld, [&](R t, bool v) { best.offer(t, v, w); });
    });
    return best.hit(sc);
}

template <typename R>
struct Blocker {
    static constexpr bool kKeys = sizeof(R) == 4 && RTC_VALU_KEYS;
    bool hit = false;
    uint32_t tmin = 0x7F800000u;
    __device__ inline void offer(R t, bool v, R dist) {
        if constexpr (kKeys) {
            const uint32_t b = __float_as_uint((v ? t : -1.0f) + 0.0f);
            tmin = b < tmin ? b : tmin;
        } else {
            hit |= v & (t >= (R)0) & (t < dist);
        }
    }
    __device__ inline bool blocked(R dist) const {
        if constexpr (kKeys) return __uint_as_float(tmin) < dist;
        else return hit;
    }
};

#ifndef RTC_SHADOW_RECTS
#define RTC_SHADOW_RECTS 1
#endif
struct NoShadowBits {
    static constexpr bool kOn = false;
    __device__ bool skips(int) const { return false; }
    __device__ bool skips_every_ball() const { return false; }
};
#ifdef RTC_JIT
template <int kPlane, int kLightIndex>
struct ShadowBits {
    static constexpr bool kOn = true;
    uint32_t w;
    __device__ inline bool skips(int caster) const {
        constexpr ShadowLayout lay{jit::kBegin, jit::kNumLights};
        const int bit = lay.pair_bit(kLightIndex, kPlane, caster);
        return bit >= 0 && ((w >> (bit & 31)) & 1u);
    }
    static constexpr uint32_t ball_mask() {
        constexpr ShadowLayout lay{jit::kBegin, jit::kNumLights};
        uint32_t m = 0;
        for (int c = 0; c < jit::kBegin[kNumKinds]; ++c)
            if (!lay.is_plane(c) && jit::kShapes[c].casts_shadow && jit::kShapes[c].bound[3] >= 0.0f &&
                jit::kShapes[c].bound[3] < __builtin_huge_valf())
                m |= 1u << lay.pair_bit(kLightIndex, kPlane, c);
        return m;
    }
    __device__ inline bool skips_every_ball() const {
        constexpr uint32_t kBalls = ball_mask();
        return (w & kBalls) == kBalls;
    }
};
#endif

template <typename R, bool kDirect = false, typename SB = NoShadowBits>
__device__ inline bool any_hit(const DevScene<R>& sc, V3<R> o, V3<R> d, R dist, V3<R> lpos, SB sb = SB{}) {
    Blocker<R> b;
#if defined(RTC_JIT) && !defined(RTC_NO_SKIPS) && RTC_SHADOW_LIGHT_CULL
    constexpr bool kLight = sizeof(R) == 4 && kDirect;
#else
    constexpr bool kLight = false;
#endif
    R dd0 = (R)0, rdd0 = (R)0;
    V3<R> rd0 = {(R)0, (R)0, (R)0};
    if constexpr (!kLight) {
        dd0 = dot(d, d);
        rdd0 = recip(dd0);
        rd0 = recip3(d);
    }
    constexpr R kLightCullFar = (R)100;
    const V3<R> tl = vsub(lpos, o);
    const R tt = Real<R>::madd(tl.z, tl.z, Real<R>::madd(tl.y, tl.y, tl.x * tl.x));
    const bool near = kLight && (sb.skips_every_ball() || !wave_any(!(tt <= kLightCullFar * kLightCullFar)));
    auto ball_may_hit = [&](R cx, R cy, R cz, R r2) {
        if (kLight && near) return wave_ball_may_hit_from<R>(cx, cy, cz, r2, lpos, tl, tt);
        return wave_ball_may_hit<R, true>(cx, cy, cz, r2, o, d, kLight ? dot(d, d) : dd0);
    };
    const bool skips = skips_on(sc);
    auto skip = [&](R cx, R cy, R cz, R r2, bool) {
        if (skips && !wave_any(!b.blocked(dist))) return true;
        if constexpr (kLight) return !ball_may_hit(cx, cy, cz, r2);
        return false;
    };
    for_all_culled<R, true, !kLight>(sc, o, d, dd0, [&]<int K>(const ShapeRec<R>& s, int slot) {
        if (!s.casts_shadow) return;
        if constexpr (SB::kOn)
            if (sb.skips(slot)) return;
        jit_fence(o, d, slot);
        if (K == RT_SHAPE_CUBE && skips) {
            const V3<R> po = xform_point(s.inv, o), pl = xform_point(s.inv, lpos);
            auto out = [](R a, R b) {
                const R lim_a = (R)1 + (R)1e-5 * ((R)1 + Real<R>::fabs(a));
                const R lim_b = (R)1 + (R)1e-5 * ((R)1 + Real<R>::fabs(b));
                return (a > lim_a && b > lim_b) || (a < -lim_a && b < -lim_b);
            };
            bool clear = out(po.x, pl.x) || out(po.y, pl.y) || out(po.z, pl.z);
            constexpr R kIn = (R)(1 - 1e-4);
            if (Real<R>::fabs(pl.x) < kIn && Real<R>::fabs(pl.y) < kIn && Real<R>::fabs(pl.z) < kIn)
                clear = clear || (Real<R>::fabs(po.x) < (R)1 && Real<R>::fabs(po.y) < (R)1 && Real<R>::fabs(po.z) < (R)1);
            if (!wave_any(!clear)) return;
        }
        if constexpr (kLight) {
            if constexpr (K != RT_SHAPE_PLANE) {
                const bool bounded = K == RT_SHAPE_SPHERE || K == RT_SHAPE_CUBE || s.bound[3] >= (R)0;
                if (bounded && !ball_may_hit(s.bound[0], s.bound[1], s.bound[2], s.bound[3])) return;
            }
        } else if (!wave_may_hit<R, K>(s, o, d, dd0)) {
            return;
        }
        if (world_sphere<R, K>(s)) {
            const R dd = kLight ? dot(d, d) : dd0;
            sphere_world<R, false>(s, o, d, dd, kLight ? recip(dd) : rdd0, [&](R t, bool v) { b.offer(t, v, dist); });
            return;
        }
        if (world_cube<R, K>(s)) {
            cube_world<R, false>(s, o, d, kLight ? recip3(d) : rd0, [&](R t, bool v) { b.offer(t, v, dist); });
            return;
        }
        const V3<R> lo = xform_point(s.inv, o);
        if (K == RT_SHAPE_PLANE && skips) {
            const R ly = xform_point(s.inv, lpos).y;
            if (!wave_any(!(lo.y * ly > (R)0 && Real<R>::fabs(lo.y) <= (R)1e4 * Real<R>::fabs(ly)))) return;
        }
        const V3<R> ld = xform_vector(s.inv, d);
        entries<R, K>(s, lo, ld, [&](R t, bool v) { b.offer(t, v, dist); });
    }, skip);
    return b.blocked(dist);
}

template <typename R, bool kDup>
__device__ inline void refractive_indices(const DevScene<R>& sc, V3<R> o, V3<R> d, const Hit<R>& h, int hit_mat,
// ... 280 lines not shown
                const R r = T::floor(T::sqrt(pp.x * pp.x + pp.z * pp.z));
                return odd_i64(r) ? v3(pr->color_b[0], pr->color_b[1], pr->color_b[2])
                                  : v3(pr->color_a[0], pr->color_a[1], pr->color_a[2]);
            }
            case RT_PATTERN_CHECKER: {
                RTC_PATTERN_KIND(RT_PATTERN_CHECKER);
                const R sum = T::floor(pp.x) + T::floor(pp.y) + T::floor(pp.z);
                return odd_i64(sum) ? v3(pr->color_b[0], pr->color_b[1], pr->color_b[2])
                                    : v3(pr->color_a[0], pr->color_a[1], pr->color_a[2]);
            }
            case RT_PATTERN_COMPLEX:
                RTC_PATTERN_KIND(RT_PATTERN_COMPLEX);
                pr = &sc.lpats[odd_i64(T::floor(pp.x)) ? pr->sub_b : pr->sub_a];
                continue;
            default:
                RTC_PATTERN_KIND(RT_PATTERN_TEST);
                return pp;
        }
    }
    return {(R)0, (R)0, (R)0};
}
template <typename R>
__device__ inline V3<R> pattern_color(const DevScene<R>& sc, int pid, const ShapeRec<R>& s, V3<R> p) {
    return pattern_color_obj(sc, pid, xform_point(s.inv, p));
}

#if !defined(RTC_JIT) && RTC_TEXTURES
template <typename R>
__device__ inline V3<R> texel_color(uint32_t t) {
    using T = Real<R>;
    return {T::div((R)(t & 0xFFu), (R)255), T::div((R)((t >> 8) & 0xFFu), (R)255), T::div((R)((t >> 16) & 0xFFu), (R)255)};
}
template <typename R>
__device__ inline V3<R> image_color(const PatternRec<R>* pr, const uint32_t* texels,
                                                        const TexRec* textures, bool have_uv, R u, R v, V3<R> obj) {
    using T = Real<R>;
    if (have_uv) {
        if (!(u >= (R)0 && u <= (R)1)) u = u - T::floor(u);
        if (!(v >= (R)0 && v <= (R)1)) v = v - T::floor(v);
    } else {
        const V3<R> pp = xform_point(pr->inv, obj);
        u = pp.x - T::floor(pp.x);
        v = pp.z - T::floor(pp.z);
    }
    const TexRec tr = textures[pr->sub_a];
    const int w1 = (int)tr.width - 1, h1 = (int)tr.height - 1;
    const uint32_t* const base = texels + tr.offset;
    const R x = u * (R)w1, y = ((R)1 - v) * (R)h1;
    const R xf = T::floor(x), yf = T::floor(y);
    const R fx = x - xf, fy = y - yf;
    const int x0 = min(max((int)xf, 0), w1), y0 = min(max((int)yf, 0), h1);
    if (pr->sub_b == RT_FILTER_NEAREST) {
        const int xi = min(x0 + (fx >= (R)0.5 ? 1 : 0), w1), yi = min(y0 + (fy >= (R)0.5 ? 1 : 0), h1);
        return texel_color<R>(base[(size_t)yi * tr.width + xi]);
    }
    const int x1 = min(x0 + 1, w1), y1 = min(y0 + 1, h1);
    const uint32_t* const r0 = base + (size_t)y0 * tr.width;
    const uint32_t* const r1 = base + (size_t)y1 * tr.width;
    const V3<R> c00 = texel_color<R>(r0[x0]), c10 = texel_color<R>(r0[x1]);
    const V3<R> c01 = texel_color<R>(r1[x0]), c11 = texel_color<R>(r1[x1]);
    const R gx = (R)1 - fx, gy = (R)1 - fy;
    return {(c00.x * gx + c10.x * fx) * gy + (c01.x * gx + c11.x * fx) * fy,
            (c00.y * gx + c10.y * fx) * gy + (c01.y * gx + c11.y * fx) * fy,
            (c00.z * gx + c10.z * fx) * gy + (c01.z * gx + c11.z * fx) * fy};
}
#endif

struct Counts {
    uint32_t c[kNumCounters];
};

__device__ inline uint32_t wave_count(bool p) {
    return (uint32_t)__builtin_popcountll(__builtin_amdgcn_ballot_w64(p));
}

template <typename R>
struct Shaded {
    V3<R> surface;
    bool refl_child = false, refr_child = false;
    bool patterned = false;
    bool refr_eval = false;
    bool schlick = false;
#if RTC_AREA_LIGHTS
    uint32_t ray_id = 0;
#endif
};

struct NoPush {
    template <typename V, typename R>
    __device__ void operator()(V, V, R) const {}
};

__device__ inline void count_generations(unsigned long long* gc, bool traced, bool shaded, uint32_t rem) {
    unsigned long long left = __builtin_amdgcn_ballot_w64(traced);
    while (left) {
        const uint32_t r = (uint32_t)__builtin_amdgcn_readlane((int)rem, (int)__builtin_ctzll(left));
        const unsigned long long same = __builtin_amdgcn_ballot_w64(traced && rem == r);
        const unsigned long long hit = __builtin_amdgcn_ballot_w64(shaded && rem == r);
        if ((threadIdx.x & 63) == 0 && r < (uint32_t)kGenSlots) {
            atomicAdd(&gc[r], (unsigned long long)__builtin_popcountll(same));
            if (hit) atomicAdd(&gc[kGenSlots + r], (unsigned long long)__builtin_popcountll(hit));
        }
        left &= ~same;
    }
}

template <typename R>
__device__ inline void count_events(Counts& k, bool primary, bool hit, const Shaded<R>& sh, int n_lights) {
#if RTC_AREA_LIGHTS
    n_lights += (int)kernarg_params<R>().area_samples;
#endif
    k.c[0] += wave_count(primary);
    const uint32_t shaded = wave_count(hit);
    k.c[4] += shaded;
    k.c[1] += shaded * (uint32_t)n_lights;
    k.c[5] += wave_count(hit & sh.patterned) * (uint32_t)n_lights;
    k.c[2] += wave_count(hit & sh.refl_child);
    k.c[3] += wave_count(hit & sh.refr_child);
    k.c[6] += wave_count(hit & sh.refr_eval);
    k.c[7] += wave_count(hit & sh.schlick);
}

template <typename R>
struct Prepared {
    V3<R> p, n, eye, over, base;
    R off;
    int mat;
};

__device__ inline int offset_class_of_kind(int kind) {
    return ((RTC_F32_FLAT_KINDS >> (kind & 31)) & 1) ? 1 : (kind == RT_SHAPE_SPHERE ? 0 : 2);
}

template <typename R>
__device__ inline int offset_class(const Hit<R>& h) {
#ifdef RTC_JIT
    if constexpr (sizeof(R) == 4) {
        int c = 2;
#pragma unroll
        for (int k = 0; k < kNumKinds; ++k)
            if (h.slot >= jit::kBegin[k] && h.slot < jit::kBegin[k + 1]) c = offset_class_of_kind(k);
        return c;
    }
#endif
    return offset_class_of_kind(h.kind);
}

template <typename R>
__device__ inline R hit_offset(const Hit<R>& h, V3<R> p, V3<R> o) {
    return Real<R>::surface_offset(p.x, p.y, p.z, o.x, o.y, o.z, offset_class(h));
}

#ifdef RTC_JIT
template <typename S>
__device__ inline void prepare_hit_const(const DevScene<float>& sc, V3<float> o, V3<float> d, const Hit<float>& h,
                                         S slot, Prepared<float>& q, bool& patterned, MaterialRec<float>& m) {
    q.p = along(o, d, h.t);
    V3<float> w = {0.0f, 0.0f, 0.0f};
    jit_record_material(slot, q.p, w, m);
    asm volatile("" : "+v"(w.x), "+v"(w.y), "+v"(w.z));
    q.n = normalized(w);
    q.eye = vneg(d);
    if (dot(q.n, q.eye) < 0.0f) q.n = vneg(q.n);
    q.mat = -1;
    int cls;
    if constexpr (S::kConst) cls = offset_class_of_kind(jit_kind_of<S::v>());
    else cls = offset_class(h);
    q.off = Real<float>::surface_offset(q.p.x, q.p.y, q.p.z, o.x, o.y, o.z, cls);
    q.over = along(q.p, q.n, q.off);
    q.base = {m.color[0], m.color[1], m.color[2]};
    patterned = m.pattern >= 0;
    if (jit::kPatterns && patterned) {
        V3<float> obj = {0.0f, 0.0f, 0.0f};
        jit_object(slot, q.over, obj);
        q.base = pattern_color_obj(sc, m.pattern, obj);
    }
}
#endif

template <typename R>
__device__ inline const MaterialRec<R>& prepare_hit(const DevScene<R>& sc, V3<R> o, V3<R> d, const Hit<R>& h,
                                                     Prepared<R>& q, bool& patterned) {
#ifdef RTC_JIT
    if constexpr (kJitRecords && sizeof(R) == 4) {
        q.p = along(o, d, h.t);
        V3<float> w = {0.0f, 0.0f, 0.0f};
        int mat = 0;
        jit_record_each<0, jit::kBegin[kNumKinds]>(h.slot, q.p, w, mat);
        asm volatile("" : "+v"(w.x), "+v"(w.y), "+v"(w.z));
        q.n = normalized(w);
        q.eye = vneg(d);
        if (dot(q.n, q.eye) < (R)0) q.n = vneg(q.n);
        q.mat = mat;
        const MaterialRec<R>& m = sc.lmats[mat];
        q.off = hit_offset(h, q.p, o);
        q.over = along(q.p, q.n, q.off);
        q.base = {m.color[0], m.color[1], m.color[2]};
        patterned = m.pattern >= 0;
        if (jit::kPatterns && patterned) {
            V3<float> obj = {0.0f, 0.0f, 0.0f};
            jit_object_each<0, jit::kBegin[kNumKinds]>(h.slot, q.over, obj);
            q.base = pattern_color_obj(sc, m.pattern, obj);
        }
        return m;
    }
#endif
#if !defined(RTC_JIT) && RTC_INSTANCES
#if RTC_TEXTURES
    {
#else
    if (kernarg_params<R>().n_instances || kernarg_params<R>().smooth_plain) {
#endif
        const LaunchParams<R>& P = kernarg_params<R>();
        const bool virt = (h.kind >> 8) != 0;
        const InstRec<R>* const I = &P.inst[virt ? (h.kind >> 8) - 1 : 0];
        const ShapeRec<R>* const g = virt ? &P.inst_shapes[h.slot] : &sc.lshapes[h.slot];
        const R* const inv = virt ? I->inv : g->inv;
        const int material = *(virt ? &I->material : &g->material);
        const int kind = h.kind & 0xFF;
        q.p = along(o, d, h.t);
        V3<R> ln;
#if RTC_TEXTURES
        R tu = (R)0, tv = (R)0;
        bool have_uv = false;
        if (kind == RT_SHAPE_TRIANGLE && (g->flags & kShapeUV)) {
            const R* const tt = virt ? P.uv_inst + (size_t)h.slot * kUVReals
                                     : P.uv_plain + (size_t)(h.slot - sc.kind_begin[RT_SHAPE_TRIANGLE]) * kUVReals;
            const TriangleTest<R> b = triangle_test(*g, xform_point(inv, o), xform_vector(inv, d));
            const R w = ((R)1 - b.u) - b.v;
            tu = (tt[2] * b.u + tt[4] * b.v) + tt[0] * w;
            tv = (tt[3] * b.u + tt[5] * b.v) + tt[1] * w;
            have_uv = true;
            if (g->flags & kShapeSmooth) {
                const R* const nn = virt ? P.smooth_inst + (size_t)h.slot * kSmoothReals
                                         : P.smooth_plain + (size_t)(h.slot - sc.kind_begin[RT_SHAPE_TRIANGLE]) * kSmoothReals;
                ln = {(nn[3] * b.u + nn[6] * b.v) + nn[0] * w, (nn[4] * b.u + nn[7] * b.v) + nn[1] * w,
                      (nn[5] * b.u + nn[8] * b.v) + nn[2] * w};
            } else {
                ln = local_normal(*g, kind, xform_point(inv, q.p));
            }
        } else
#endif
        if (kind == RT_SHAPE_TRIANGLE && (g->flags & kShapeSmooth)) {
            const R* const nn = virt ? P.smooth_inst + (size_t)h.slot * kSmoothReals
                                     : P.smooth_plain + (size_t)(h.slot - sc.kind_begin[RT_SHAPE_TRIANGLE]) * kSmoothReals;
            const TriangleTest<R> b = triangle_test(*g, xform_point(inv, o), xform_vector(inv, d));
            const R w = ((R)1 - b.u) - b.v;
            ln = {(nn[3] * b.u + nn[6] * b.v) + nn[0] * w, (nn[4] * b.u + nn[7] * b.v) + nn[1] * w,
                  (nn[5] * b.u + nn[8] * b.v) + nn[2] * w};
        } else {
            ln = local_normal(*g, kind, xform_point(inv, q.p));
        }
        q.n = normalized(xform_normal(inv, ln));
        q.eye = vneg(d);
        if (dot(q.n, q.eye) < (R)0) q.n = vneg(q.n);
        q.mat = material;
        const MaterialRec<R>& m = sc.lmats[material];
        q.off = hit_offset(h, q.p, o);
        q.over = along(q.p, q.n, q.off);
        q.base = {m.color[0], m.color[1], m.color[2]};
        patterned = m.pattern >= 0;
#if RTC_TEXTURES
        if (patterned) {
            const PatternRec<R>* const pr = &sc.lpats[m.pattern];
            if (P.textures && pr->kind == RT_PATTERN_IMAGE)
                q.base = image_color<R>(pr, P.texels, P.textures, have_uv, tu, tv, xform_point(inv, q.over));
            else
                q.base = pattern_color_obj(sc, m.pattern, xform_point(inv, q.over));
        }
#else
        if (patterned) q.base = pattern_color_obj(sc, m.pattern, xform_point(inv, q.over));
#endif
        return m;
    }
#endif
    const ShapeRec<R>& s = sc.lshapes[h.slot];
    q.p = along(o, d, h.t);
    q.n = hit_normal(s, h.slot, h.kind, q.p);
    q.eye = vneg(d);
    if (dot(q.n, q.eye) < (R)0) q.n = vneg(q.n);
    q.mat = s.material;
    const MaterialRec<R>& m = sc.lmats[s.material];
    q.off = hit_offset(h, q.p, o);
        q.over = along(q.p, q.n, q.off);
    q.base = {m.color[0], m.color[1], m.color[2]};
    patterned = m.pattern >= 0;
#ifdef RTC_JIT
    constexpr bool kPatterns = jit::kPatterns;
#else
    constexpr bool kPatterns = true;
#endif
    if (kPatterns && patterned) q.base = pattern_color(sc, m.pattern, s, q.over);
    return m;
}

#ifdef RTC_JIT
template <int I, int E, typename F>
__device__ inline void jit_light_each(F&& f) {
    if constexpr (I < E) {
        f(jit::kLights[I]);
        jit_light_each<I + 1, E>(f);
    }
}
#endif
template <typename R, typename F>
__device__ inline void for_lights(const DevScene<R>& sc, F&& f) {
#ifdef RTC_JIT
    if constexpr (sizeof(R) == 4) {
        jit_light_each<0, jit::kNumLights>(f);
        return;
    }
#endif
    for (int li = 0; li < sc.n_lights; ++li) f(ld_uniform(&sc.lights[li]));
}

template <typename R>
__device__ inline V3<R> lighting_term(const LightRec<R>& L, const MaterialRec<R>& m, V3<R> base, V3<R> n, V3<R> eye,
                                      V3<R> ld, R ldn, bool shadowed) {
    const V3<R> eff = {base.x * L.intensity[0], base.y * L.intensity[1], base.z * L.intensity[2]};
    V3<R> c = {eff.x * m.ambient, eff.y * m.ambient, eff.z * m.ambient};
    if (!shadowed) {
        if (!(ldn < (R)0)) {
            c = {c.x + (eff.x * m.diffuse) * ldn, c.y + (eff.y * m.diffuse) * ldn, c.z + (eff.z * m.diffuse) * ldn};
            if (m.specular != (R)0) {
                const R rde = dot(reflect(vneg(ld), n), eye);
                if (!(rde <= (R)0)) {
                    const R f = Real<R>::pow(rde, m.shininess);
                    c = {c.x + (L.intensity[0] * m.specular) * f, c.y + (L.intensity[1] * m.specular) * f,
                         c.z + (L.intensity[2] * m.specular) * f};
                }
            }
        }
    }
    return c;
}

template <typename R>
struct LightSide {
    V3<R> ld;
    R ldn;
    bool shadowed;
};
template <typename R, bool kDirect, typename SB = NoShadowBits>
__device__ __attribute__((always_inline)) inline LightSide<R> light_side(const DevScene<R>& sc, const LightRec<R>& L,
                                                                         V3<R> over, V3<R> n, SB sb = SB{}) {
    const V3<R> lpos = {L.position[0], L.position[1], L.position[2]};
    const V3<R> to_light = vsub(lpos, over);
    const R dist = magnitude(to_light);
    const V3<R> ld = normalized(to_light);
    const R ldn = dot(ld, n);
    bool shadowed = false;
    if (!(ldn < (R)0) || !skips_on(sc)) shadowed = any_hit<R, kDirect, SB>(sc, over, ld, dist, lpos, sb);
    return {ld, ldn, shadowed};
}

#if RTC_AREA_LIGHTS
__device__ inline uint32_t area_mix(uint32_t x) {
    x ^= x >> 16;
    x *= 0x7feb352du;
    x ^= x >> 15;
    x *= 0x846ca68bu;
    x ^= x >> 16;
    return x;
}

struct AreaPassBits {
    static constexpr bool kOn = true;
    unsigned long long pass;
    __device__ inline bool skips(int slot) const { return slot >= 0 && slot < 64 && ((pass >> slot) & 1ull); }
    __device__ inline bool skips_every_ball() const { return false; }
};
template <typename R>
__device__ inline unsigned long long area_pass_mask(const DevScene<R>& sc, const AreaLightRec<R>& A, uint32_t us,
                                                    uint32_t vs, V3<R> over) {
    const R fu = (R)us, fv = (R)vs;
    const V3<R> U = {A.uvec[0] * fu, A.uvec[1] * fu, A.uvec[2] * fu};
    const V3<R> V = {A.vvec[0] * fv, A.vvec[1] * fv, A.vvec[2] * fv};
    const V3<R> lc = {A.corner[0] + (U.x + V.x) * (R)0.5, A.corner[1] + (U.y + V.y) * (R)0.5,
                      A.corner[2] + (U.z + V.z) * (R)0.5};
    const R lr = (magnitude(U) + magnitude(V)) * (R)0.5;
    const V3<R> w = vsub(lc, over);
    const R ww = dot(w, w), rww = recip(ww);
    const int n_slots = sc.kind_begin[kNumKinds] < 64 ? sc.kind_begin[kNumKinds] : 64;
    unsigned long long pass = 0;
    for (int slot = 0; slot < n_slots; ++slot) {
        const ShapeRec<R>* s = &sc.shapes[slot];
        const R r2 = s->bound[3];
        if (!(r2 >= (R)0) || !(r2 < Real<R>::kInf)) continue;
        const R reach = Real<R>::sqrt(r2) + lr;
        const V3<R> v = {s->bound[0] - over.x, s->bound[1] - over.y, s->bound[2] - over.z};
        const R vv = dot(v, v);
        R t = dot(v, w) * rww;
        t = t < (R)0 ? (R)0 : (t > (R)1 ? (R)1 : t);
        const V3<R> e = {v.x - t * w.x, v.y - t * w.y, v.z - t * w.z};
        const bool far = dot(e, e) > (reach * reach) * (R)1.001 + (R)1e-4 * (vv + ww);
        if (!wave_any(!far)) pass |= 1ull << slot;
    }
    return pass;
}

template <typename R, bool kDirect>
__device__ inline V3<R> area_light_term(const DevScene<R>& sc, const AreaLightRec<R>& A, uint32_t area_index,
                                        uint32_t ray_id, uint32_t remaining, const MaterialRec<R>& m, V3<R> base,
                                        V3<R> n, V3<R> eye, V3<R> over) {
    const uint32_t us = A.usteps < (uint32_t)RT_LIGHT_MAX_STEPS ? A.usteps : (uint32_t)RT_LIGHT_MAX_STEPS;
    const uint32_t vs = A.vsteps < (uint32_t)RT_LIGHT_MAX_STEPS ? A.vsteps : (uint32_t)RT_LIGHT_MAX_STEPS;
    const V3<R> eff = {base.x * A.intensity[0], base.y * A.intensity[1], base.z * A.intensity[2]};
    const V3<R> kd = {eff.x * m.diffuse, eff.y * m.diffuse, eff.z * m.diffuse};
    const V3<R> ks = {A.intensity[0] * m.specular, A.intensity[1] * m.specular, A.intensity[2] * m.specular};
    const uint32_t key0 = area_mix(area_mix(A.seed ^ ray_id) ^ remaining);
    const AreaPassBits sb{kernarg_params<R>().area_cull && skips_on(sc) ? area_pass_mask(sc, A, us, vs, over) : 0ull};
    V3<R> sum = {(R)0, (R)0, (R)0};
    uint32_t k = 0;
    for (uint32_t j = 0; j < vs; ++j) {
        for (uint32_t i = 0; i < us; ++i, ++k) {
            R ju = (R)0.5, jv = (R)0.5;
            if (A.jitter == RT_JITTER_HASHED) {
                const uint32_t key = area_mix(key0 ^ ((area_index << 8) | k));
                ju = (R)(key >> 8) * (R)5.9604644775390625e-8;
                jv = (R)(area_mix(key ^ 0x9E3779B9u) >> 8) * (R)5.9604644775390625e-8;
            }
            const R fu = (R)i + ju, fv = (R)j + jv;
            LightRec<R> L;
            for (int q = 0; q < 3; ++q) {
                L.position[q] = (A.corner[q] + A.uvec[q] * fu) + A.vvec[q] * fv;
                L.intensity[q] = A.intensity[q];
            }
            const LightSide<R> s = light_side<R, kDirect, AreaPassBits>(sc, L, over, n, sb);
            if (!s.shadowed && !(s.ldn < (R)0)) {
                V3<R> c = {kd.x * s.ldn, kd.y * s.ldn, kd.z * s.ldn};
                if (m.specular != (R)0) {
                    const R rde = dot(reflect(vneg(s.ld), n), eye);
                    if (!(rde <= (R)0)) {
                        const R f = Real<R>::pow(rde, m.shininess);
                        c = {c.x + ks.x * f, c.y + ks.y * f, c.z + ks.z * f};
                    }
                }
                sum = {sum.x + c.x, sum.y + c.y, sum.z + c.z};
            }
        }
    }
    const R nn = (R)(us * vs);
    return {eff.x * m.ambient + Real<R>::div(sum.x, nn), eff.y * m.ambient + Real<R>::div(sum.y, nn),
            eff.z * m.ambient + Real<R>::div(sum.z, nn)};
}
#endif

#ifdef RTC_JIT
template <int I, int E, int kPlane, typename F>
__device__ inline void jit_light_each_bits(uint32_t w, F&& f) {
    if constexpr (I < E) {
        f(jit::kLights[I], ShadowBits<kPlane, I>{w});
        jit_light_each_bits<I + 1, E, kPlane>(w, f);
    }
}
template <bool kDirect, typename S>
__device__ __attribute__((always_inline)) inline void shade_hit_const(const DevScene<float>& sc, V3<float> o, V3<float> d,
                                                                      const Hit<float>& h, S slot, Shaded<float>& out,
                                                                      uint32_t miss = 0u) {
    Prepared<float> q;
    MaterialRec<float> m;
    prepare_hit_const(sc, o, d, h, slot, q, out.patterned, m);
    V3<float> surface = {0.0f, 0.0f, 0.0f};
    auto light = [&](const LightRec<float>& L, auto sb) {
        const LightSide<float> s = light_side<float, kDirect>(sc, L, q.over, q.n, sb);
        const V3<float> c = lighting_term(L, m, q.base, q.n, q.eye, s.ld, s.ldn, s.shadowed);
        surface = {surface.x + c.x, surface.y + c.y, surface.z + c.z};
    };
    constexpr ShadowLayout kLay{jit::kBegin, jit::kNumLights};
    constexpr int kSlot = [] { if constexpr (S::kConst) return S::v; else return -1; }();
#if !defined(RTC_NO_SKIPS) && RTC_SHADOW_RECTS
    constexpr bool kBits = kDirect && kSlot >= 0 && kLay.fits() && kLay.is_plane(kSlot);
#else
    constexpr bool kBits = false;
#endif
    if constexpr (kBits) {
        constexpr uint32_t kNear = 1u << kLay.near_bit(kSlot);
        const uint32_t w = miss & kNear ? miss : 0u;
        jit_light_each_bits<0, jit::kNumLights, kSlot>(w, light);
    } else {
        (void)miss;
        for_lights(sc, [&](const LightRec<float>& L) { light(L, NoShadowBits{}); });
    }
    out.surface = surface;
    out.refl_child = out.refr_child = false;
    out.schlick = (m.reflectiveness > 0.0f) & (m.transparency > 0.0f);
}
#endif

template <typename R, bool kChildren, bool kDup = false, typename Push = NoPush, typename B = NoBlock>
__device__ inline bool shade_ray(const DevScene<R>& sc, V3<R> o, V3<R> d, uint32_t remaining, Shaded<R>& out,
                                 Push&& push = Push{}, B blk = B{}) {
    using T = Real<R>;
    const Hit<R> h = closest_hit(sc, o, d, blk);
    if (h.slot < 0) return false;
#ifdef RTC_JIT
    if constexpr (kJitConstMaterials && !kChildren && sizeof(R) == 4) {
#if !defined(RTC_NO_SKIPS) && RTC_UNIFORM_HIT
        if constexpr (B::kOn && jit::kBegin[kNumKinds] <= kUniformHitSlots) {
            const int first = __builtin_amdgcn_readfirstlane(h.slot);
            if (!wave_any(h.slot != first)) {
                jit_slot_ladder<0, jit::kBegin[kNumKinds]>(
                    first, [&](auto slot) { shade_hit_const<B::kOn>(sc, o, d, h, slot, out, blk.miss); });
                return true;
            }
        }
#endif
        shade_hit_const<B::kOn>(sc, o, d, h, LaneSlot{h.slot}, out);
        return true;
    }
#endif
    Prepared<R> q;
    const MaterialRec<R>& m = prepare_hit(sc, o, d, h, q, out.patterned);
    const V3<R> p = q.p, n = q.n, eye = q.eye, over = q.over, base = q.base;
    const R off = q.off;
    V3<R> surface = {(R)0, (R)0, (R)0};
    for_lights(sc, [&](const LightRec<R>& L) {
        const LightSide<R> s = light_side<R, B::kOn>(sc, L, over, n);
        const V3<R> c = lighting_term(L, m, base, n, eye, s.ld, s.ldn, s.shadowed);
        surface = {surface.x + c.x, surface.y + c.y, surface.z + c.z};
    });
#if RTC_AREA_LIGHTS
    {
        const LaunchParams<R>& AP = kernarg_params<R>();
        const uint32_t n_area = AP.area ? AP.n_area : 0u;
        for (uint32_t ai = 0; ai < n_area; ++ai) {
            const AreaLightRec<R> A = ld_const(&AP.area[ai]);
            const V3<R> c = area_light_term<R, B::kOn>(sc, A, ai, out.ray_id, remaining, m, base, n, eye, over);
            surface = {surface.x + c.x, surface.y + c.y, surface.z + c.z};
        }
    }
#endif
    out.surface = surface;
    out.refl_child = out.refr_child = false;
    out.schlick = (m.reflectiveness > (R)0) & (m.transparency > (R)0);
    if constexpr (kChildren) {
#ifdef RTC_JIT
        constexpr bool kTransparent = jit::kTransparent;
#else
        constexpr bool kTransparent = true;
#endif
        const bool reflective = m.reflectiveness > (R)0, transparent = kTransparent && m.transparency > (R)0;
        R n1 = (R)1, n2 = (R)1;
        if (kTransparent && m.transparency != (R)0 && remaining > 0)
            refractive_indices<R, kDup>(sc, o, d, h, q.mat, n1, n2);
        R fr = (R)1, ft = (R)1;
        if (reflective && transparent) {
            R cs = dot(eye, n);
            bool total = false;
            if (n1 > n2) {
                const R ratio = T::div(n1, n2);
                const R sin2 = (ratio * ratio) * ((R)1 - cs * cs);
                if (sin2 > (R)1) total = true;
                else cs = T::sqrt((R)1 - sin2);
            }
            R rr = (R)1;
            if (!total) {
                const R q = T::div(n1 - n2, n1 + n2);
                const R r0 = q * q;
                const R x = (R)1 - cs;
                rr = T::rfma((R)1 - r0, x * ((x * x) * (x * x)), r0);
            }
            fr = rr;
            ft = (R)1 - rr;
        }
        if (remaining > 0 && m.reflectiveness != (R)0) {
            out.refl_child = true;
            push(over, reflect(d, n), m.reflectiveness * fr);
        }
        if (kTransparent && remaining > 0 && m.transparency != (R)0) {
            out.refr_eval = true;
            const R nr = T::div(n1, n2);
            const R cos_i = dot(eye, n);
            const R sin2_t = (nr * nr) * ((R)1 - cos_i * cos_i);
            if (!(sin2_t > (R)1)) {
                const R cos_t = T::sqrt((R)1 - sin2_t);
                const R f = T::rfma(nr, cos_i, -cos_t);
                out.refr_child = true;
                push(along(p, n, -off),
                     V3<R>{n.x * f - eye.x * nr, n.y * f - eye.y * nr, n.z * f - eye.z * nr}, m.transparency * ft);
            }
        }
    }
    return true;
}

template <typename R>
__device__ inline void camera_ray(const CameraRec<R>& c, uint32_t x, uint32_t y, V3<R>& o, V3<R>& d) {
    const R ox = ((R)x + (R)0.5) * c.pixel_size;
    const R oy = ((R)y + (R)0.5) * c.pixel_size;
    const R wx = c.half_width - ox;
    const R wy = c.half_height - oy;
    o = {c.origin[0], c.origin[1], c.origin[2]};
    if constexpr (sizeof(R) == 4) {
        d = normalized(xform_vector(c.inv, V3<R>{wx, wy, (R)-1}));
    } else {
        const V3<R> pixel = xform_point(c.inv, V3<R>{wx, wy, (R)-1});
        d = normalized(vsub(pixel, o));
    }
}

template <typename R>
__device__ inline void store_pixel(const LaunchParams<R>& P, uint64_t idx, V3<R> c) {
    if (P.out_format == RT_OUT_U8) {
        auto q = [](R v) -> uint8_t {
            if (!(v == v)) return 0;
            v = v < (R)0 ? (R)0 : (v > (R)1 ? (R)1 : v);
            if constexpr (sizeof(R) == 4) return (uint8_t)__builtin_roundf(v * (R)255);
            else return (uint8_t)__builtin_round(v * (R)255);
        };
        uint8_t* o = static_cast<uint8_t*>(P.out) + 3 * idx;
        __builtin_nontemporal_store(q(c.x), o);
        __builtin_nontemporal_store(q(c.y), o + 1);
        __builtin_nontemporal_store(q(c.z), o + 2);
    } else {
        R* o = static_cast<R*>(P.out) + 3 * idx;
        __builtin_nontemporal_store(c.x, o);
        __builtin_nontemporal_store(c.y, o + 1);
        __builtin_nontemporal_store(c.z, o + 2);
    }
}

#ifndef RTC_WAVE_W
#define RTC_WAVE_W 16
#endif
static_assert(RT_TILE_W % RTC_WAVE_W == 0 && RT_TILE_H % (64 / RTC_WAVE_W) == 0, "the 4 waves tile the tile");
template <typename R>
__device__ inline bool tile_pixel(const LaunchParams<R>& P, uint32_t t, uint32_t tid, uint32_t& x, uint32_t& y,
                                  uint64_t& out_idx) {
    const uint32_t lrow = div_by(t, P.tiles_x, P.tiles_x_magic), tcol = t - lrow * P.tiles_x;
    constexpr uint32_t kPerRow = RT_TILE_W / RTC_WAVE_W, kWaveH = 64 / RTC_WAVE_W;
    const uint32_t wave = tid / 64, lane = tid % 64;
    const uint32_t local_y = lrow * RT_TILE_H + (wave / kPerRow) * kWaveH + lane / RTC_WAVE_W;
    x = tcol * RT_TILE_W + (wave % kPerRow) * RTC_WAVE_W + lane % RTC_WAVE_W;
    y = shard_image_row(local_y, P.shard_count, P.shard_index);
    out_idx = (uint64_t)(P.image_rows ? y : local_y) * P.width + x;
    return x < P.width && y < P.height;
}

#ifdef RTC_JIT
template <typename R>
__device__ inline PixelBlock wave_pixel_block(const LaunchParams<R>& P, uint32_t t) {
    constexpr uint32_t kPerRow = RT_TILE_W / RTC_WAVE_W, kWaveH = 64 / RTC_WAVE_W;
    if constexpr (RTC_WAVE_W != kCullCellW || kWaveH != kCullCellH || RT_TILE_H % kCullCellH != 0) return {0u};
    const uint32_t lrow = div_by(t, P.tiles_x, P.tiles_x_magic), tcol = t - lrow * P.tiles_x;
    const uint32_t wave = __builtin_amdgcn_readfirstlane(threadIdx.x / 64);
    const uint32_t row0 = lrow * RT_TILE_H + (wave / kPerRow) * kWaveH;
    const uint32_t cx = tcol * (RT_TILE_W / kCullCellW) + wave % kPerRow;
    const uint32_t cy = shard_image_row(row0, P.shard_count, P.shard_index) / kCullCellH;
    static_assert((kCullCols & (kCullCols - 1)) == 0 && (kCullRows & (kCullRows - 1)) == 0);
    return {P.cull_cols[cx & (kCullCols - 1)] | P.cull_rows[cy & (kCullRows - 1)]};
}
#endif

template <typename R, bool kFramesOnly = false>
__device__ inline void load_primary(const LaunchParams<R>& P, uint32_t t, uint32_t tid, bool& valid, V3<R>& o,
                                    V3<R>& d, uint64_t& out_idx) {
    if (!kFramesOnly && P.rays) {
        const uint64_t r = (uint64_t)t * kBlock + tid;
        valid = r < P.n_rays;
        out_idx = r;
        if (valid) {
            const double* q = P.rays + 6 * r;
            o = {(R)q[0], (R)q[1], (R)q[2]};
            d = {(R)q[3], (R)q[4], (R)q[5]};
        }
    } else {
        uint32_t x, y;
        valid = tile_pixel(P, t, tid, x, y, out_idx);
        if (valid) camera_ray(P.cam, x, y, o, d);
    }
}

#if RTC_AREA_LIGHTS
template <typename R>
__device__ inline uint32_t primary_ray_id(const LaunchParams<R>& P, uint32_t t, uint32_t lane) {
    if (P.rays) return (uint32_t)((uint64_t)t * kBlock + lane);
    uint32_t x, y;
    uint64_t out_idx;
    (void)tile_pixel(P, t, lane, x, y, out_idx);
    return y * P.width + x;
}
template <typename R>
__device__ inline uint32_t sample_ray_id(const LaunchParams<R>& P, uint32_t t, uint32_t lane, uint32_t n, uint32_t i,
                                         uint32_t j) {
    uint32_t x, y;
    uint64_t out_idx;
    (void)tile_pixel(P, t, lane, x, y, out_idx);
    return (n * y + j) * (n * P.width) + n * x + i;
}
#endif

__device__ inline void flush_counts(const Counts& k, unsigned long long* global) {
    __shared__ uint32_t s_counts[kBlock / 64][kNumCounters];
    const uint32_t wave = threadIdx.x / 64, lane = threadIdx.x % 64;
    if (lane == 0)
        for (int i = 0; i < kNumCounters; ++i) s_counts[wave][i] = k.c[i];
    __syncthreads();
    if (threadIdx.x < (uint32_t)kNumCounters) {
        unsigned long long v = 0;
        for (uint32_t w = 0; w < kBlock / 64; ++w) v += s_counts[w][threadIdx.x];
        const uint32_t shard = blockIdx.x % kCounterShards;
        if (v) atomicAdd(&global[shard * kNumCounters + threadIdx.x], v);
    }
}

template <typename R>
__device__ inline unsigned int next_tile(const LaunchParams<R>& P, uint32_t it, uint32_t& probe, uint32_t n_items) {
    if (P.persistent == kSchedGrid) return it == 0 ? blockIdx.x : kNoItem;
    if (P.persistent == kSchedStatic) {
        const unsigned long long t = blockIdx.x + (unsigned long long)it * gridDim.x;
        return t < P.n_tiles ? (unsigned int)t : kNoItem;
    }
    for (; probe < (uint32_t)kTileQueues; ++probe) {
        const uint32_t q = (blockIdx.x + probe) % kTileQueues;
        const unsigned long long j = atomicAdd(&P.tile_counter[q * kQueueStride], 1ull);
        const unsigned long long i = q + (unsigned long long)kTileQueues * j;
        if (i < n_items) return P.tile_order ? P.tile_order[i] : (unsigned int)i;
    }
    return kNoItem;
}

template <typename R, bool kLds>
__device__ inline DevScene<R> scene_view(const LaunchParams<R>& P, const ShapeRec<R>* __restrict__ shapes,
                                         const MaterialRec<R>* __restrict__ materials,
                                         const PatternRec<R>* __restrict__ patterns,
                                         const LightRec<R>* __restrict__ lights, unsigned char* smem,
                                         bool stage = false) {
    DevScene<R> sc = P.scene;
    sc.no_skips = (P.flags & RT_FLAG_NO_SKIPS) != 0;
    sc.shapes = shapes;
    sc.materials = materials;
    sc.patterns = patterns;
    sc.lights = lights;
    if constexpr (kLds && kJitRecords && sizeof(R) == 4) {
        auto* lm = reinterpret_cast<MaterialRec<R>*>(smem);
        auto* lp = reinterpret_cast<PatternRec<R>*>(lm + sc.n_materials);
        if (stage) {
            const uint4* s4 = reinterpret_cast<const uint4*>(materials);
            uint4* d4 = reinterpret_cast<uint4*>(lm);
            for (uint32_t i = threadIdx.x; i < P.world_lds / 16; i += kBlock) d4[i] = s4[i];
            __syncthreads();
        }
        sc.lshapes = shapes;
        sc.lmats = lm;
        sc.lpats = lp;
        sc.lworld_slot = sc.world_slot;
    } else if constexpr (kLds) {
        const int ns = sc.kind_begin[kNumKinds];
        auto* ls = reinterpret_cast<ShapeRec<R>*>(smem);
        auto* lm = reinterpret_cast<MaterialRec<R>*>(ls + ns);
        auto* lp = reinterpret_cast<PatternRec<R>*>(lm + sc.n_materials);
        auto* lw = reinterpret_cast<int32_t*>(lp + sc.n_patterns);
        if (stage) {
            const uint4* s4 = reinterpret_cast<const uint4*>(shapes);
            uint4* d4 = reinterpret_cast<uint4*>(ls);
            for (uint32_t i = threadIdx.x; i < P.world_lds / 16; i += kBlock) d4[i] = s4[i];
            __syncthreads();
        }
        sc.lworld_slot = lw;
        sc.lshapes = ls;
        sc.lmats = lm;
        sc.lpats = lp;
    } else {
        sc.lshapes = shapes;
        sc.lmats = materials;
        sc.lpats = patterns;
        sc.lworld_slot = sc.world_slot;
    }
    return sc;
}

template <typename R>
__device__ inline const LaunchParams<R>& kernarg_params() {
    auto k = __builtin_amdgcn_kernarg_segment_ptr();
    asm volatile("" : "+s"(k));
    return *(const LaunchParams<R>*)k;
}

#define RTC_WORLD_PARAMS(R)                                                                                  \
    const ShapeRec<R>* __restrict__ shapes, const MaterialRec<R>* __restrict__ materials,                   \
        const PatternRec<R>* __restrict__ patterns, const LightRec<R>* __restrict__ lights

#ifndef RTC_DIRECT_WAVES
#define RTC_DIRECT_WAVES 8
#endif
#ifndef RTC_POOL_WAVES
#define RTC_POOL_WAVES 6
#endif
template <typename R, bool kLds>
__global__ __launch_bounds__(kBlock) __attribute__((amdgpu_waves_per_eu(sizeof(R) == 4 ? RTC_DIRECT_WAVES : 1))) void trace_direct(
    LaunchParams<R> P, RTC_WORLD_PARAMS(R)) {
    extern __shared__ __align__(16) unsigned char smem[];
    (void)scene_view<R, kLds>(P, shapes, materials, patterns, lights, smem, true);
#ifdef RTC_JIT
    constexpr bool kDiag = false;
#else
    const bool kDiag = true;
#endif
    if (kDiag && P.stamps && threadIdx.x == 0) P.stamps[2 * blockIdx.x] = __builtin_amdgcn_s_memrealtime();
    Counts k = {};
    const uint32_t tid = threadIdx.x;
    for (uint32_t t = blockIdx.x;; t += gridDim.x) {
        const LaunchParams<R>& P = kernarg_params<R>();
        const DevScene<R> sc = scene_view<R, kLds>(P, shapes, materials, patterns, lights, smem);
        if (t >= P.n_tiles) break;
        bool valid;
        V3<R> o, d;
        uint64_t out_idx;
#ifdef RTC_JIT
        load_primary<R, true>(P, t, tid, valid, o, d, out_idx);
#else
        load_primary(P, t, tid, valid, o, d, out_idx);
#endif
        V3<R> c = {(R)0, (R)0, (R)0};
        Shaded<R> sh;
        bool hit = false;
#if RTC_AREA_LIGHTS
        sh.ray_id = primary_ray_id(P, t, tid);
#endif
        if (valid) {
            if (kDiag && (P.flags & (RT_FLAG_NO_SHADE | RT_FLAG_NO_TRACE))) {
                if (P.flags & RT_FLAG_NO_TRACE) {
                    c = d;
                } else {
                    const Hit<R> h = closest_hit(sc, o, d);
                    c = {h.t * (R)0.01, (R)h.slot, (R)0};
                }
#ifdef RTC_JIT
            } else if (shade_ray<R, false>(sc, o, d, 0, sh, NoPush{}, wave_pixel_block(P, t))) {
#elif RTC_AREA_LIGHTS
            } else if (shade_ray<R, false>(sc, o, d, P.max_depth, sh)) {
#else
            } else if (shade_ray<R, false>(sc, o, d, 0, sh)) {
#endif
                hit = true;
                c = sh.surface;
            }
        }
        count_events(k, valid, hit, sh, sc.n_lights);
        if (kDiag && P.gen_counts) count_generations(P.gen_counts, valid, hit, P.max_depth);
        if (valid) store_pixel(P, out_idx, c);
    }
    if (!(P.flags & RT_FLAG_NO_COUNTERS)) flush_counts(k, P.counters);
    if (kDiag && P.stamps) {
        __syncthreads();
        if (threadIdx.x == 0) P.stamps[2 * blockIdx.x + 1] = __builtin_amdgcn_s_memrealtime();
    }
}

__device__ inline void set_wave_prio(uint32_t p) {
    if (p == 0) __builtin_amdgcn_s_setprio(0);
    else if (p == 1) __builtin_amdgcn_s_setprio(1);
    else if (p == 2) __builtin_amdgcn_s_setprio(2);
    else __builtin_amdgcn_s_setprio(3);
}

template <typename R>
struct Pool {
    PoolAcc<R>* acc;
    R* lds;
    R* spill;
    int lds_cap, spill_cap;
#ifdef RTC_BOUNDS_CHECK
    int32_t* err;
#endif
};

__device__ inline bool in_bounds(bool ok, int32_t* err, int32_t bit) {
#ifdef RTC_BOUNDS_CHECK
    if (!ok) atomicOr(err, bit);
    return ok;
#else
    (void)err;
    (void)bit;
    (void)ok;
    return true;
#endif
}

__device__ inline int wave_reserve(bool pred, int* top) {
    const unsigned long long m = __builtin_amdgcn_ballot_w64(pred);
    if (m == 0) return -1;
    const int prefix = __builtin_amdgcn_mbcnt_hi((unsigned)(m >> 32), __builtin_amdgcn_mbcnt_lo((unsigned)m, 0u));
    const int leader = __ffsll((long long)m) - 1;
    int base = 0;
    if ((int)(threadIdx.x & 63) == leader) base = atomicAdd(top, __popcll(m));
    base = __shfl(base, leader);
    return pred ? base + prefix : -1;
}

#define RTC_AS_LDS __attribute__((address_space(3)))
#define RTC_AS_GLOBAL __attribute__((address_space(1)))

template <typename R, typename PR, typename PU>
__device__ inline void pool_store(PR base, PU metas, int n, int i, V3<R> o, V3<R> d, R w, uint32_t meta) {
    base[i] = o.x;
    base[n + i] = o.y;
    base[2 * n + i] = o.z;
    base[3 * n + i] = d.x;
    base[4 * n + i] = d.y;
    base[5 * n + i] = d.z;
    base[6 * n + i] = w;
    metas[i] = meta;
}

template <typename R, typename PR, typename PU>
__device__ inline void pool_load(PR base, PU metas, int n, int i, V3<R>& o, V3<R>& d, R& w, uint32_t& meta) {
    o = {base[i], base[n + i], base[2 * n + i]};
    d = {base[3 * n + i], base[4 * n + i], base[5 * n + i]};
    w = base[6 * n + i];
    meta = metas[i];
}

template <typename R>
__device__ inline void spill_store(RTC_AS_GLOBAL R* e, V3<R> o, V3<R> d, R w, uint32_t meta) {
    if constexpr (sizeof(R) == 4) {
        typedef float f4 __attribute__((ext_vector_type(4)));
        RTC_AS_GLOBAL f4* p = (RTC_AS_GLOBAL f4*)e;
        p[0] = f4{o.x, o.y, o.z, d.x};
        p[1] = f4{d.y, d.z, w, __uint_as_float(meta)};
    } else {
        typedef double d2 __attribute__((ext_vector_type(2)));
        RTC_AS_GLOBAL d2* p = (RTC_AS_GLOBAL d2*)e;
        p[0] = d2{o.x, o.y};
        p[1] = d2{o.z, d.x};
        p[2] = d2{d.y, d.z};
        p[3] = d2{w, __longlong_as_double((long long)meta)};
    }
}

template <typename R>
__device__ inline void spill_load(const RTC_AS_GLOBAL R* e, V3<R>& o, V3<R>& d, R& w, uint32_t& meta) {
    if constexpr (sizeof(R) == 4) {
        typedef float f4 __attribute__((ext_vector_type(4)));
        const RTC_AS_GLOBAL f4* p = (const RTC_AS_GLOBAL f4*)e;
        const f4 a = p[0], b = p[1];
        o = {a.x, a.y, a.z};
        d = {a.w, b.x, b.y};
        w = b.z;
        meta = __float_as_uint(b.w);
    } else {
        typedef double d2 __attribute__((ext_vector_type(2)));
        const RTC_AS_GLOBAL d2* p = (const RTC_AS_GLOBAL d2*)e;
        const d2 a = p[0], b = p[1], c = p[2], q = p[3];
        o = {a.x, a.y, b.x};
        d = {b.y, c.x, c.y};
        w = q.x;
        meta = (uint32_t)__double_as_longlong(q.y);
    }
}

template <typename R>
__device__ inline void pool_put(const Pool<R>& pl, int slot, V3<R> o, V3<R> d, R w, uint32_t meta) {
#ifdef RTC_BOUNDS_CHECK
    if (!in_bounds(slot >= 0 && slot < pl.lds_cap + pl.spill_cap, pl.err, kErrBoundsSlot)) return;
#endif
    if (slot < pl.lds_cap) {
        RTC_AS_LDS R* b = (RTC_AS_LDS R*)pl.lds;
        pool_store<R>(b, (RTC_AS_LDS PoolMeta*)(b + 7 * pl.lds_cap), pl.lds_cap, slot, o, d, w, meta);
    } else {
        spill_store<R>((RTC_AS_GLOBAL R*)pl.spill + 8 * (size_t)(slot - pl.lds_cap), o, d, w, meta);
    }
}

template <typename R>
__device__ inline void pool_get(const Pool<R>& pl, int slot, V3<R>& o, V3<R>& d, R& w, uint32_t& meta) {
#ifdef RTC_BOUNDS_CHECK
    if (!in_bounds(slot >= 0 && slot < pl.lds_cap + pl.spill_cap, pl.err, kErrBoundsSlot)) {
        o = d = {(R)0, (R)0, (R)0};
        w = (R)0;
        meta = 0;
        return;
    }
#endif
    if (slot < pl.lds_cap) {
        const RTC_AS_LDS R* b = (const RTC_AS_LDS R*)pl.lds;
        pool_load<R>(b, (const RTC_AS_LDS PoolMeta*)(b + 7 * pl.lds_cap), pl.lds_cap, slot, o, d, w, meta);
    } else {
        spill_load<R>((const RTC_AS_GLOBAL R*)pl.spill + 8 * (size_t)(slot - pl.lds_cap), o, d, w, meta);
    }
}

// ... 633 lines not shown
        } else {
            if (dup) RTC_LAUNCH(trace_pool, false, true);
            else RTC_LAUNCH(trace_pool, false, false);
        }
#endif
    } else {
#ifdef RTC_POOL_ONLY
        return hipErrorInvalidValue;
#else
        if (lds) RTC_LAUNCH(trace_direct, true);
        else RTC_LAUNCH(trace_direct, false);
#endif
    }
#undef RTC_LAUNCH
    return hipGetLastError();
}

template <typename R>
hipError_t occupancy(bool pool, bool lds, size_t dyn_lds, int* blocks_per_cu) {
    if (pool)
        return lds ? hipOccupancyMaxActiveBlocksPerMultiprocessor(blocks_per_cu, trace_pool<R, true, false>, kBlock,
                                                                  dyn_lds)
                   : hipOccupancyMaxActiveBlocksPerMultiprocessor(blocks_per_cu, trace_pool<R, false, false>, kBlock,
                                                                  dyn_lds);
#ifdef RTC_POOL_ONLY
    return hipErrorInvalidValue;
#endif
    return lds ? hipOccupancyMaxActiveBlocksPerMultiprocessor(blocks_per_cu, trace_direct<R, true>, kBlock, dyn_lds)
               : hipOccupancyMaxActiveBlocksPerMultiprocessor(blocks_per_cu, trace_direct<R, false>, kBlock, dyn_lds);
}

#if RTC_PRECISION != 2
template hipError_t launch_trace<float>(const LaunchParams<float>&, bool, bool, uint32_t, size_t, hipStream_t);
template hipError_t occupancy<float>(bool, bool, size_t, int*);
#endif
#ifndef RTC_POOL_ONLY
#if RTC_PRECISION != 1
template hipError_t launch_trace<double>(const LaunchParams<double>&, bool, bool, uint32_t, size_t, hipStream_t);
template hipError_t occupancy<double>(bool, bool, size_t, int*);
#endif

template <typename R>
hipError_t launch_trace_rays(const LaunchParams<R>& P, bool dup, uint32_t grid, size_t dyn_lds, const void* rays,
                             void* rgb, void* hits, hipStream_t stream) {
    (void)hipGetLastError();
    const RayBatch<R> B{static_cast<const R*>(rays), static_cast<R*>(rgb), hits};
#define RTC_LAUNCH(...)                                                                                      \
    hipLaunchKernelGGL((trace_rays<R, __VA_ARGS__>), dim3(grid), dim3(kBlock), dyn_lds, stream, P, P.scene.shapes, \
                       P.scene.materials, P.scene.patterns, P.scene.lights, B)
    if (P.world_lds != 0) {
        if (dup) RTC_LAUNCH(true, true);
        else RTC_LAUNCH(true, false);
    } else {
        if (dup) RTC_LAUNCH(false, true);
        else RTC_LAUNCH(false, false);
    }
#undef RTC_LAUNCH
    return hipGetLastError();
}

template <typename R>
hipError_t occupancy_rays(bool lds, size_t dyn_lds, int* blocks_per_cu) {
    return lds ? hipOccupancyMaxActiveBlocksPerMultiprocessor(blocks_per_cu, trace_rays<R, true, false>, kBlock, dyn_lds)
               : hipOccupancyMaxActiveBlocksPerMultiprocessor(blocks_per_cu, trace_rays<R, false, false>, kBlock,
                                                              dyn_lds);
}
#if RTC_PRECISION != 2
template hipError_t launch_trace_rays<float>(const LaunchParams<float>&, bool, uint32_t, size_t, const void*, void*,
                                             void*, hipStream_t);
template hipError_t occupancy_rays<float>(bool, size_t, int*);
#endif
#if RTC_PRECISION != 1
template hipError_t launch_trace_rays<double>(const LaunchParams<double>&, bool, uint32_t, size_t, const void*, void*,
                                              void*, hipStream_t);
template hipError_t occupancy_rays<double>(bool, size_t, int*);
#endif

template <typename R>
hipError_t launch_trace_ss(const LaunchParams<R>& P, bool pool, bool dup, uint32_t grid, size_t dyn_lds,
                           hipStream_t stream) {
    (void)hipGetLastError();
    const bool lds = P.world_lds != 0;
#define RTC_LAUNCH(K, ...)                                                                                \
    hipLaunchKernelGGL((K<R, __VA_ARGS__>), dim3(grid), dim3(kBlock), dyn_lds, stream, P, P.scene.shapes,         \
                       P.scene.materials, P.scene.patterns, P.scene.lights)
    if (pool) {
        if (lds) {
            if (dup) RTC_LAUNCH(trace_pool_ss, true, true);
            else RTC_LAUNCH(trace_pool_ss, true, false);
        } else {
            if (dup) RTC_LAUNCH(trace_pool_ss, false, true);
            else RTC_LAUNCH(trace_pool_ss, false, false);
        }
    } else {
        if (lds) RTC_LAUNCH(trace_direct_ss, true);
        else RTC_LAUNCH(trace_direct_ss, false);
    }
#undef RTC_LAUNCH
    return hipGetLastError();
}

template <typename R>
hipError_t occupancy_ss(bool pool, bool lds, size_t dyn_lds, int* blocks_per_cu) {
    if (pool)
        return lds ? hipOccupancyMaxActiveBlocksPerMultiprocessor(blocks_per_cu, trace_pool_ss<R, true, false>, kBlock,
                                                                  dyn_lds)
                   : hipOccupancyMaxActiveBlocksPerMultiprocessor(blocks_per_cu, trace_pool_ss<R, false, false>,
                                                                  kBlock, dyn_lds);
    return lds ? hipOccupancyMaxActiveBlocksPerMultiprocessor(blocks_per_cu, trace_direct_ss<R, true>, kBlock, dyn_lds)
               : hipOccupancyMaxActiveBlocksPerMultiprocessor(blocks_per_cu, trace_direct_ss<R, false>, kBlock,
                                                              dyn_lds);
}
#if RTC_PRECISION != 2
template hipError_t launch_trace_ss<float>(const LaunchParams<float>&, bool, bool, uint32_t, size_t, hipStream_t);
template hipError_t occupancy_ss<float>(bool, bool, size_t, int*);
#endif
#if RTC_PRECISION != 1
template hipError_t launch_trace_ss<double>(const LaunchParams<double>&, bool, bool, uint32_t, size_t, hipStream_t);
template hipError_t occupancy_ss<double>(bool, bool, size_t, int*);
#endif

#if RTC_PRECISION != 2 && !RTC_INSTANCES
hipError_t launch_order_tiles(uint32_t* cost, uint32_t* order, uint32_t n, uint32_t* n_items, float split_per_cost,
                              uint32_t max_split_log2, float urgent_per_cost, uint32_t graded, uint32_t min_split_log2,
                              hipStream_t stream) {
    (void)hipGetLastError();
    hipLaunchKernelGGL(order_tiles, dim3(1), dim3(kOrderThreads), 0, stream, cost, order, n, n_items, split_per_cost,
                       max_split_log2, urgent_per_cost, graded, min_split_log2);
    return hipGetLastError();
}
#endif

#if !RTC_INSTANCES
template <typename R>
hipError_t launch_debug_shape(const ShapeRec<R>* shapes, int slot, int kind, uint32_t mode, uint32_t world_space,
                              const double* in, uint32_t n, double* out, hipStream_t stream) {
    (void)hipGetLastError();
    hipLaunchKernelGGL(debug_shape<R>, dim3((n + 255) / 256), dim3(256), 0, stream, shapes, slot, kind, mode,
                       world_space, in, n, out);
    return hipGetLastError();
}
#if RTC_PRECISION != 2
template hipError_t launch_debug_shape<float>(const ShapeRec<float>*, int, int, uint32_t, uint32_t, const double*,
                                              uint32_t, double*, hipStream_t);
#endif
#if RTC_PRECISION != 1
template hipError_t launch_debug_shape<double>(const ShapeRec<double>*, int, int, uint32_t, uint32_t, const double*,
                                               uint32_t, double*, hipStream_t);
#endif

#endif

#if RTC_PRECISION != 2 && !RTC_INSTANCES
hipError_t launch_canvas_signal(unsigned long long* flag, unsigned long long seq, hipStream_t stream) {
    (void)hipGetLastError();
    hipLaunchKernelGGL(canvas_signal, dim3(1), dim3(64), 0, stream, flag, seq);
    return hipGetLastError();
}
hipError_t launch_canvas_wait(const unsigned long long* flags, uint32_t n, unsigned long long seq,
                              unsigned long long timeout_ticks, int32_t* err, hipStream_t stream) {
    (void)hipGetLastError();
    hipLaunchKernelGGL(canvas_wait, dim3(1), dim3(64), 0, stream, flags, n, seq, timeout_ticks, err);
    return hipGetLastError();
}
#endif

#if RTC_PRECISION != 2 && !RTC_INSTANCES
hipError_t launch_assemble(const void* gathered, void* image, uint32_t width, uint32_t height, uint32_t shards,
                           uint32_t strip_rows, uint32_t bpp, hipStream_t stream) {
    (void)hipGetLastError();
    const uint64_t row_bytes = (uint64_t)width * bpp;
    const bool wide = ((row_bytes | (uintptr_t)gathered | (uintptr_t)image) & 15) == 0;
    const uint64_t per_row = wide ? (row_bytes / 16 + 255) / 256 : 4;
    dim3 grid((uint32_t)std::min<uint64_t>(std::max<uint64_t>(per_row, 1), 64), height);
    hipLaunchKernelGGL(assemble_shards, grid, dim3(256), 0, stream, static_cast<const unsigned char*>(gathered),
                       static_cast<unsigned char*>(image), width, height, shards, strip_rows, bpp);
    return hipGetLastError();
}
#endif

#endif
#endif
#ifdef RTC_VARIANT
}
#endif
}
```

Baseline: 446,700 Mray/s.

## Precompute plane heights, unit normals and origin terms per launch for direct kernel

Per-scene plane normals are normalized once on the GPU at JIT time and baked into the generated header, which removes the per-hit normalization for constant plane slots. Per-launch host terms (camera origin max-abs and the camera height in each plane's local frame) are added to LaunchParams and loaded into scalar registers. These replace the per-ray plane origin transform and the origin-based surface offset. The tile decode is also simplified with a per-wave tile helper that reuses the cull-cell lookup. The cost is more launch-parameter bytes and scalar registers, plus reliance on every primary ray sharing the camera origin.

```diff
diff --git a/profiles/jit/three_sphere_direct.hpp b/profiles/jit/three_sphere_direct.hpp
--- a/profiles/jit/three_sphere_direct.hpp
+++ b/profiles/jit/three_sphere_direct.hpp
@@ -31,5 +31,14 @@
 constexpr bool kPatterns = false;
 constexpr uint32_t kPatternKinds = 0u;
 constexpr bool kTransparent = false;
+#define RTC_JIT_UNIT_NORMALS 1
+constexpr float kUnitNormal[7][3] = {
+    {__builtin_bit_cast(float, 0x00000000u), __builtin_bit_cast(float, 0x00000000u), __builtin_bit_cast(float, 0x00000000u)},
+    {__builtin_bit_cast(float, 0x00000000u), __builtin_bit_cast(float, 0x00000000u), __builtin_bit_cast(float, 0x00000000u)},
+    {__builtin_bit_cast(float, 0x00000000u), __builtin_bit_cast(float, 0x00000000u), __builtin_bit_cast(float, 0x00000000u)},
+    {__builtin_bit_cast(float, 0x00000000u), __builtin_bit_cast(float, 0x3f800000u), __builtin_bit_cast(float, 0x00000000u)},
+    {__builtin_bit_cast(float, 0xbf2e930eu), __builtin_bit_cast(float, 0xb676812fu), __builtin_bit_cast(float, 0x3f3b3e17u)},
+    {__builtin_bit_cast(float, 0x3f2e930eu), __builtin_bit_cast(float, 0xb676812fu), __builtin_bit_cast(float, 0x3f3b3e17u)},
+    {}};
 }
 }
diff --git a/ray-tracer-challenge-rs_amd/csrc/launch_terms.hpp b/ray-tracer-challenge-rs_amd/csrc/launch_terms.hpp
--- /dev/null
+++ b/ray-tracer-challenge-rs_amd/csrc/launch_terms.hpp
@@ -0,0 +1,24 @@
+#pragma once
+
+#include <cmath>
+#include <cstdint>
+#include <cstring>
+
+#include "rtc_internal.hpp"
+
+namespace rtc {
+
+inline float launch_kfma(float m, float x, float acc) { return m == 0.0f ? acc : std::fmaf(m, x, acc); }
+
+inline void launch_terms(const ShapeRec<float>* shapes, const int32_t* kind_begin, int n, const float origin[3],
+                         LaunchTerms& out) {
+    std::memset(&out, 0, sizeof out);
+    out.head[0] = std::fmax(std::fmax(std::fabs(origin[0]), std::fabs(origin[1])), std::fabs(origin[2]));
+    const int p0 = kind_begin[RT_SHAPE_PLANE], p1 = kind_begin[RT_SHAPE_PLANE + 1];
+    for (int s = p0; s < p1 && s < n && s < kPrimaryRectSlots; ++s) {
+        const float* m = shapes[s].inv;
+        out.head[1 + s - p0] = launch_kfma(m[6], origin[2], launch_kfma(m[5], origin[1], launch_kfma(m[4], origin[0], m[7])));
+    }
+}
+
+}
diff --git a/ray-tracer-challenge-rs_amd/csrc/rtc_host.cpp b/ray-tracer-challenge-rs_amd/csrc/rtc_host.cpp
--- a/ray-tracer-challenge-rs_amd/csrc/rtc_host.cpp
+++ b/ray-tracer-challenge-rs_amd/csrc/rtc_host.cpp
@@ -15,6 +15,7 @@
 #include "flop_model.hpp"
 #include "host_math.hpp"
 #include "debug_knobs.hpp"
+#include "launch_terms.hpp"
 #include "primary_rect.hpp"
 #include "rtc_context.hpp"
 #include "rtc_internal.hpp"
@@ -871,8 +872,10 @@
     if (flags & RT_FLAG_FAIL_LAUNCH) return set_error(RT_ERR_HIP, "launch refused (RT_FLAG_FAIL_LAUNCH)");
     if constexpr (sizeof(R) == 4) {
         const size_t ns = ctx->jit.shapes.size();
-        if (jf && !ls.pool && cam && !ss && ns <= (size_t)kPrimaryRectSlots && (int)ns == w.scene.kind_begin[kNumKinds] &&
-            P.width <= kCullCols * kCullCellW && P.height <= kCullRows * kCullCellH) {
+        const bool small_direct = jf && !ls.pool && cam && !ss && ns <= (size_t)kPrimaryRectSlots &&
+                                  (int)ns == w.scene.kind_begin[kNumKinds];
+        if (small_direct) launch_terms(ctx->jit.shapes.data(), w.scene.kind_begin, (int)ns, P.cam.origin, P.terms);
+        if (small_direct && P.width <= kCullCols * kCullCellW && P.height <= kCullRows * kCullCellH) {
             const uint32_t nc = (P.width + kCullCellW - 1) / kCullCellW, nr = (P.height + kCullCellH - 1) / kCullCellH;
             uint32_t flip_cols[kCullCols + 1] = {}, flip_rows[kCullRows + 1] = {};
             auto outside = [&](const uint32_t r[4], uint32_t b) {
diff --git a/ray-tracer-challenge-rs_amd/csrc/rtc_internal.hpp b/ray-tracer-challenge-rs_amd/csrc/rtc_internal.hpp
--- a/ray-tracer-challenge-rs_amd/csrc/rtc_internal.hpp
+++ b/ray-tracer-challenge-rs_amd/csrc/rtc_internal.hpp
@@ -23,8 +23,11 @@
     const uint32_t trows = (height + RT_TILE_H - 1) / RT_TILE_H;
     return trows > shard ? (trows - shard + shards - 1) / shards : 0;
 }
+RTC_HD inline uint32_t shard_tile_image_row(uint32_t tile_row, uint32_t shards, uint32_t shard) {
+    return (tile_row * shards + shard) * RT_TILE_H;
+}
 RTC_HD inline uint32_t shard_image_row(uint32_t strip_row, uint32_t shards, uint32_t shard) {
-    return ((strip_row / RT_TILE_H) * shards + shard) * RT_TILE_H + strip_row % RT_TILE_H;
+    return shard_tile_image_row(strip_row / RT_TILE_H, shards, shard) + strip_row % RT_TILE_H;
 }
 RTC_HD inline void shard_of_image_row(uint32_t y, uint32_t shards, uint32_t* shard, uint32_t* strip_row) {
     const uint32_t trow = y / RT_TILE_H;
@@ -304,6 +307,10 @@
         const int rank = c == slot ? casters : (c < plane0 ? c : c - planes);
         return kShadowBit0 + planes + (light * planes + (slot - plane0)) * (casters + 1) + rank;
     }
+};
+
+struct alignas(16) LaunchTerms {
+    float head[kPrimaryRectSlots + 4];
 };
 
 template <typename R>
@@ -363,6 +370,8 @@
     uint32_t n_area;
     uint32_t area_samples;
     uint32_t area_cull;
-};
-
-}
+    LaunchTerms terms;
+};
+static_assert(sizeof(LaunchParams<float>) + 4 * sizeof(void*) <= 4096 && sizeof(LaunchParams<double>) + 4 * sizeof(void*) <= 4096);
+
+}
diff --git a/ray-tracer-challenge-rs_amd/csrc/rtc_jit.cpp b/ray-tracer-challenge-rs_amd/csrc/rtc_jit.cpp
--- a/ray-tracer-challenge-rs_amd/csrc/rtc_jit.cpp
+++ b/ray-tracer-challenge-rs_amd/csrc/rtc_jit.cpp
@@ -35,6 +35,8 @@
 extern char** environ;
 
 namespace rtc {
+
+hipError_t launch_unit_vectors(const float* in, float* out, uint32_t n, hipStream_t stream);
 
 struct CodeBuild {
     std::atomic<int> state{0};
@@ -214,7 +216,7 @@
 
 std::string scene_header(const std::vector<ShapeRec<float>>& sh, const int32_t begin[kNumKinds + 1],
                          const std::vector<LightRec<float>>& lights, const std::vector<MaterialRec<float>>& mats,
-                         bool patterns, uint32_t pattern_kinds, bool transparent) {
+                         bool patterns, uint32_t pattern_kinds, bool transparent, const std::vector<float>& unit) {
     std::string s = "#pragma once\n#include \"rtc_internal.hpp\"\nnamespace rtc {\nnamespace jit {\n";
     s += "constexpr int kBegin[" + std::to_string(kNumKinds + 1) + "] = {";
     for (int k = 0; k <= kNumKinds; ++k) s += (k ? ", " : "") + std::to_string(begin[k]);
@@ -255,8 +257,42 @@
     s += std::string("constexpr bool kPatterns = ") + (patterns ? "true" : "false") + ";\n";
     s += "constexpr uint32_t kPatternKinds = " + std::to_string(pattern_kinds) + "u;\n";
     s += std::string("constexpr bool kTransparent = ") + (transparent ? "true" : "false") + ";\n";
+    if (unit.size() == 3 * sh.size() && !sh.empty()) {
+        s += "#define RTC_JIT_UNIT_NORMALS 1\nconstexpr float kUnitNormal[" + std::to_string(sh.size() + 1) + "][3] = {\n";
+        for (size_t i = 0; i < sh.size(); ++i)
+            s += "    {" + hexf(unit[3 * i]) + ", " + hexf(unit[3 * i + 1]) + ", " + hexf(unit[3 * i + 2]) + "},\n";
+        s += "    {}};\n";
+    }
     s += "}  // namespace jit\n}  // namespace rtc\n";
     return s;
+}
+
+std::vector<float> unit_normals(rt_context* ctx) {
+    const std::vector<ShapeRec<float>>& sh = ctx->jit.shapes;
+    const int p0 = ctx->jit.begin[RT_SHAPE_PLANE], p1 = ctx->jit.begin[RT_SHAPE_PLANE + 1];
+    if (p1 <= p0 || sh.size() > 64) return {};
+    auto kmul = [](float m, float x) { return m == 0.0f ? 0.0f : m * x; };
+    auto kfma = [](float m, float x, float acc) { return m == 0.0f ? acc : std::fmaf(m, x, acc); };
+    std::vector<float> w(3 * sh.size(), 0.0f), out(3 * sh.size(), 0.0f);
+    for (int s = p0; s < p1; ++s)
+        for (int c = 0; c < 3; ++c)
+            w[3 * s + c] = kfma(sh[s].inv[8 + c], 0.0f, kfma(sh[s].inv[4 + c], 1.0f, kmul(sh[s].inv[c], 0.0f)));
+    const size_t bytes = w.size() * sizeof(float);
+    float* d = nullptr;
+    bool ok = hipSetDevice(ctx->device) == hipSuccess && hipMalloc(&d, 2 * bytes) == hipSuccess;
+    if (ok) {
+        ok = hipMemcpy(d, w.data(), bytes, hipMemcpyHostToDevice) == hipSuccess &&
+             launch_unit_vectors(d, d + w.size(), (uint32_t)sh.size(), nullptr) == hipSuccess &&
+             hipMemcpy(out.data(), d + w.size(), bytes, hipMemcpyDeviceToHost) == hipSuccess;
+        (void)hipFree(d);
+    }
+    if (!ok) {
+        (void)hipGetLastError();
+        return {};
+    }
+    for (int s = 0; s < (int)sh.size(); ++s)
+        if (s < p0 || s >= p1) out[3 * s] = out[3 * s + 1] = out[3 * s + 2] = 0.0f;
+    return out;
 }
 
 const char* kernel_name(bool pool, bool lds, bool ss) {
@@ -529,10 +565,11 @@
         if (start) {
             ctx->jit.owner[variant] = true;
             uint64_t key = 0;
+            const std::vector<float> unit = !pool && !ss ? unit_normals(ctx) : std::vector<float>();
             const jitfile::Request rq =
                 make_request(scene_header(ctx->jit.shapes, ctx->jit.begin, ctx->jit.lights, ctx->jit.materials,
                                           ctx->jit.patterns,
-                                          ctx->jit.pattern_kinds, ctx->jit.transparent),
+                                          ctx->jit.pattern_kinds, ctx->jit.transparent, unit),
                              kernel_name(pool, lds, ss), device_arch(ctx), &key, no_skips, pool_waves);
             start_build(b, rq, key, sync && !start_only);
         }
diff --git a/ray-tracer-challenge-rs_amd/csrc/rtc_kernels.hip b/ray-tracer-challenge-rs_amd/csrc/rtc_kernels.hip
--- a/ray-tracer-challenge-rs_amd/csrc/rtc_kernels.hip
+++ b/ray-tracer-challenge-rs_amd/csrc/rtc_kernels.hip
@@ -650,6 +650,13 @@
             asm volatile("" : "+v"(o.x), "+v"(o.y), "+v"(o.z), "+v"(d.x), "+v"(d.y), "+v"(d.z));
 #endif
 }
+template <typename R>
+__device__ inline void jit_fence_dir(V3<R>& d, int slot = 0) {
+#if defined(RTC_JIT) && !defined(RTC_JIT_NO_FENCE)
+    if constexpr (sizeof(R) == 4 && jit::kBegin[kNumKinds] >= RTC_JIT_FENCE_MIN_SHAPES)
+        if (slot % RTC_JIT_FENCE_EVERY == 0) asm volatile("" : "+v"(d.x), "+v"(d.y), "+v"(d.z));
+#endif
+}
 
 #ifdef RTC_JIT
 constexpr int jit_kind_of(int slot) {
@@ -815,11 +822,26 @@
 struct NoBlock {
     static constexpr bool kOn = false;
     __device__ bool misses(int) const { return false; }
+    __device__ float plane_height(int) const { return 0.0f; }
+    __device__ float origin_max() const { return 0.0f; }
 };
+#ifndef RTC_LAUNCH_TERMS
+#define RTC_LAUNCH_TERMS 1
+#endif
+#ifdef RTC_JIT
+constexpr int kJitPlane0 = jit::kBegin[RT_SHAPE_PLANE];
+constexpr int kJitPlanes = jit::kBegin[RT_SHAPE_PLANE + 1] - kJitPlane0;
+#else
+constexpr int kJitPlane0 = 0, kJitPlanes = 0;
+#endif
 struct PixelBlock {
     static constexpr bool kOn = true;
     uint32_t miss;
     __device__ inline bool misses(int slot) const { return (miss >> slot) & 1u; }
+    static constexpr int kHead = kJitPlanes <= kPrimaryRectSlots ? (1 + kJitPlanes + 3) / 4 * 4 : 4;
+    float head[kHead];
+    __device__ inline float plane_height(int plane) const { return head[1 + plane]; }
+    __device__ inline float origin_max() const { return head[0]; }
 };
 
 template <typename R, typename B = NoBlock>
@@ -831,6 +853,11 @@
 #else
     constexpr bool kRects = false, kLazy = false;
 #endif
+#if defined(RTC_JIT) && RTC_LAUNCH_TERMS
+    constexpr bool kTerms = B::kOn && sizeof(R) == 4 && jit::kBegin[kNumKinds] <= kPrimaryRectSlots;
+#else
+    constexpr bool kTerms = false;
+#endif
     R dd0 = (R)0, rdd0 = (R)0;
     V3<R> rd0 = {(R)0, (R)0, (R)0};
     if constexpr (!kLazy) {
@@ -839,7 +866,8 @@
         rd0 = recip3(d);
     }
     for_all_culled<R, true>(sc, o, d, dd0, [&]<int K>(const ShapeRec<R>& s, int slot) {
-        jit_fence(o, d, slot);
+        if constexpr (kTerms) jit_fence_dir(d, slot);
+        else jit_fence(o, d, slot);
         if constexpr (kRects && K != RT_SHAPE_PLANE)
             if (blk.misses(slot)) return;
         const R dd = kLazy ? dot(d, d) : dd0;
@@ -855,7 +883,9 @@
             cube_world<R, true>(s, o, d, rd, [&](R t, bool v) { best.offer(t, v, w); });
             return;
         }
-        const V3<R> lo = xform_point(s.inv, o);
+        V3<R> lo = {(R)0, (R)0, (R)0};
+        if constexpr (kTerms && K == RT_SHAPE_PLANE) lo.y = blk.plane_height(slot - kJitPlane0);
+        else lo = xform_point(s.inv, o);
         const V3<R> ld = xform_vector(s.inv, d);
         if (K == RT_SHAPE_PLANE && skips_on(sc)) {
             if (!wave_any(!(lo.y * ld.y > (R)0))) return;
@@ -1442,21 +1472,41 @@
 }
 
 #ifdef RTC_JIT
-template <typename S>
+#ifndef RTC_UNIT_NORMALS
+#define RTC_UNIT_NORMALS 1
+#endif
+template <bool kDirect, typename S>
 __device__ inline void prepare_hit_const(const DevScene<float>& sc, V3<float> o, V3<float> d, const Hit<float>& h,
-                                         S slot, Prepared<float>& q, bool& patterned, MaterialRec<float>& m) {
+                                         S slot, Prepared<float>& q, bool& patterned, MaterialRec<float>& m,
+                                         float origin_max = 0.0f) {
     q.p = along(o, d, h.t);
     V3<float> w = {0.0f, 0.0f, 0.0f};
     jit_record_material(slot, q.p, w, m);
-    asm volatile("" : "+v"(w.x), "+v"(w.y), "+v"(w.z));
-    q.n = normalized(w);
+#if defined(RTC_JIT_UNIT_NORMALS) && RTC_UNIT_NORMALS
+    constexpr int kPlaneSlot = [] {
+        if constexpr (S::kConst) return jit_kind_of<S::v>() == RT_SHAPE_PLANE ? S::v : -1;
+        else return -1;
+    }();
+    if constexpr (kPlaneSlot >= 0) {
+        q.n = {jit::kUnitNormal[kPlaneSlot][0], jit::kUnitNormal[kPlaneSlot][1], jit::kUnitNormal[kPlaneSlot][2]};
+    } else
+#endif
+    {
+        asm volatile("" : "+v"(w.x), "+v"(w.y), "+v"(w.z));
+        q.n = normalized(w);
+    }
     q.eye = vneg(d);
     if (dot(q.n, q.eye) < 0.0f) q.n = vneg(q.n);
     q.mat = -1;
     int cls;
     if constexpr (S::kConst) cls = offset_class_of_kind(jit_kind_of<S::v>());
     else cls = offset_class(h);
-    q.off = Real<float>::surface_offset(q.p.x, q.p.y, q.p.z, o.x, o.y, o.z, cls);
+#if RTC_LAUNCH_TERMS
+    if constexpr (kDirect && jit::kBegin[kNumKinds] <= kPrimaryRectSlots) {
+        q.off = Real<float>::surface_offset(q.p.x, q.p.y, q.p.z, origin_max, origin_max, origin_max, cls);
+    } else
+#endif
+        q.off = Real<float>::surface_offset(q.p.x, q.p.y, q.p.z, o.x, o.y, o.z, cls);
     q.over = along(q.p, q.n, q.off);
     q.base = {m.color[0], m.color[1], m.color[2]};
     patterned = m.pattern >= 0;
@@ -1747,10 +1797,10 @@
 template <bool kDirect, typename S>
 __device__ __attribute__((always_inline)) inline void shade_hit_const(const DevScene<float>& sc, V3<float> o, V3<float> d,
                                                                       const Hit<float>& h, S slot, Shaded<float>& out,
-                                                                      uint32_t miss = 0u) {
+                                                                      uint32_t miss = 0u, float origin_max = 0.0f) {
     Prepared<float> q;
     MaterialRec<float> m;
-    prepare_hit_const(sc, o, d, h, slot, q, out.patterned, m);
+    prepare_hit_const<kDirect>(sc, o, d, h, slot, q, out.patterned, m, origin_max);
     V3<float> surface = {0.0f, 0.0f, 0.0f};
     auto light = [&](const LightRec<float>& L, auto sb) {
         const LightSide<float> s = light_side<float, kDirect>(sc, L, q.over, q.n, sb);
@@ -1791,12 +1841,12 @@
             const int first = __builtin_amdgcn_readfirstlane(h.slot);
             if (!wave_any(h.slot != first)) {
                 jit_slot_ladder<0, jit::kBegin[kNumKinds]>(
-                    first, [&](auto slot) { shade_hit_const<B::kOn>(sc, o, d, h, slot, out, blk.miss); });
+                    first, [&](auto slot) { shade_hit_const<B::kOn>(sc, o, d, h, slot, out, blk.miss, blk.origin_max()); });
                 return true;
             }
         }
 #endif
-        shade_hit_const<B::kOn>(sc, o, d, h, LaneSlot{h.slot}, out);
+        shade_hit_const<B::kOn>(sc, o, d, h, LaneSlot{h.slot}, out, 0u, blk.origin_max());
         return true;
     }
 #endif
@@ -1915,10 +1965,19 @@
 #define RTC_WAVE_W 16
 #endif
 static_assert(RT_TILE_W % RTC_WAVE_W == 0 && RT_TILE_H % (64 / RTC_WAVE_W) == 0, "the 4 waves tile the tile");
+struct TileAt {
+    uint32_t lrow, tcol;
+};
+template <typename R>
+__device__ inline TileAt tile_at(const LaunchParams<R>& P, uint32_t t) {
+    const uint32_t lrow = div_by(t, P.tiles_x, P.tiles_x_magic);
+    return {lrow, t - lrow * P.tiles_x};
+}
 template <typename R>
 __device__ inline bool tile_pixel(const LaunchParams<R>& P, uint32_t t, uint32_t tid, uint32_t& x, uint32_t& y,
                                   uint64_t& out_idx) {
-    const uint32_t lrow = div_by(t, P.tiles_x, P.tiles_x_magic), tcol = t - lrow * P.tiles_x;
+    const TileAt at = tile_at(P, t);
+    const uint32_t lrow = at.lrow, tcol = at.tcol;
     constexpr uint32_t kPerRow = RT_TILE_W / RTC_WAVE_W, kWaveH = 64 / RTC_WAVE_W;
     const uint32_t wave = tid / 64, lane = tid % 64;
     const uint32_t local_y = lrow * RT_TILE_H + (wave / kPerRow) * kWaveH + lane / RTC_WAVE_W;
@@ -1929,17 +1988,44 @@
 }
 
 #ifdef RTC_JIT
-template <typename R>
-__device__ inline PixelBlock wave_pixel_block(const LaunchParams<R>& P, uint32_t t) {
+struct WaveTile {
+    uint32_t x0;
+    uint32_t row0;
+    uint32_t y0;
+};
+template <typename R>
+__device__ inline WaveTile wave_tile(const LaunchParams<R>& P, uint32_t t) {
     constexpr uint32_t kPerRow = RT_TILE_W / RTC_WAVE_W, kWaveH = 64 / RTC_WAVE_W;
-    if constexpr (RTC_WAVE_W != kCullCellW || kWaveH != kCullCellH || RT_TILE_H % kCullCellH != 0) return {0u};
-    const uint32_t lrow = div_by(t, P.tiles_x, P.tiles_x_magic), tcol = t - lrow * P.tiles_x;
+    const TileAt at = tile_at(P, t);
     const uint32_t wave = __builtin_amdgcn_readfirstlane(threadIdx.x / 64);
-    const uint32_t row0 = lrow * RT_TILE_H + (wave / kPerRow) * kWaveH;
-    const uint32_t cx = tcol * (RT_TILE_W / kCullCellW) + wave % kPerRow;
-    const uint32_t cy = shard_image_row(row0, P.shard_count, P.shard_index) / kCullCellH;
+    const uint32_t wrow = (wave / kPerRow) * kWaveH;
+    return {at.tcol * RT_TILE_W + (wave % kPerRow) * RTC_WAVE_W, at.lrow * RT_TILE_H + wrow,
+            shard_tile_image_row(at.lrow, P.shard_count, P.shard_index) + wrow};
+}
+template <typename R>
+__device__ inline bool wave_tile_pixel(const LaunchParams<R>& P, const WaveTile& w, uint32_t lane, uint32_t& x,
+                                       uint32_t& y, uint64_t& out_idx) {
+    const uint32_t ly = lane / RTC_WAVE_W;
+    x = w.x0 + lane % RTC_WAVE_W;
+    y = w.y0 + ly;
+    out_idx = (uint64_t)((P.image_rows ? w.y0 : w.row0) + ly) * P.width + x;
+    return x < P.width && y < P.height;
+}
+template <typename R>
+__device__ inline PixelBlock wave_pixel_block(const LaunchParams<R>& P, const WaveTile& w) {
+    constexpr uint32_t kWaveH = 64 / RTC_WAVE_W;
+    PixelBlock block = {0u, {}};
+    constexpr bool kHeights = RTC_LAUNCH_TERMS && sizeof(R) == 4 && jit::kBegin[kNumKinds] <= kPrimaryRectSlots;
+    if constexpr (kHeights)
+        for (int i = 0; i < PixelBlock::kHead; ++i) block.head[i] = P.terms.head[i];
+    if constexpr (RTC_WAVE_W != kCullCellW || kWaveH != kCullCellH || RT_TILE_H % kCullCellH != 0) return block;
+    const uint32_t cx = w.x0 / kCullCellW, cy = w.y0 / kCullCellH;
     static_assert((kCullCols & (kCullCols - 1)) == 0 && (kCullRows & (kCullRows - 1)) == 0);
-    return {P.cull_cols[cx & (kCullCols - 1)] | P.cull_rows[cy & (kCullRows - 1)]};
+    block.miss = P.cull_cols[cx & (kCullCols - 1)] | P.cull_rows[cy & (kCullRows - 1)];
+    asm volatile("" : "+s"(block.miss));
+    if constexpr (kHeights)
+        for (int i = 0; i < PixelBlock::kHead; ++i) asm volatile("" : "+s"(block.head[i]));
+    return block;
 }
 #endif
 
@@ -2078,6 +2164,9 @@
 #ifndef RTC_POOL_WAVES
 #define RTC_POOL_WAVES 6
 #endif
+#ifndef RTC_TILE_DECODE
+#define RTC_TILE_DECODE 1
+#endif
 template <typename R, bool kLds>
 __global__ __launch_bounds__(kBlock) __attribute__((amdgpu_waves_per_eu(sizeof(R) == 4 ? RTC_DIRECT_WAVES : 1))) void trace_direct(
     LaunchParams<R> P, RTC_WORLD_PARAMS(R)) {
@@ -2099,7 +2188,17 @@
         V3<R> o, d;
         uint64_t out_idx;
 #ifdef RTC_JIT
+#if RTC_TILE_DECODE
+        const WaveTile wt = wave_tile(P, t);
+        {
+            uint32_t x, y;
+            valid = wave_tile_pixel(P, wt, tid % 64, x, y, out_idx);
+            if (valid) camera_ray(P.cam, x, y, o, d);
+            o = {P.cam.origin[0], P.cam.origin[1], P.cam.origin[2]};
+        }
+#else
         load_primary<R, true>(P, t, tid, valid, o, d, out_idx);
+#endif
 #else
         load_primary(P, t, tid, valid, o, d, out_idx);
 #endif
@@ -2118,7 +2217,11 @@
                     c = {h.t * (R)0.01, (R)h.slot, (R)0};
                 }
 #ifdef RTC_JIT
-            } else if (shade_ray<R, false>(sc, o, d, 0, sh, NoPush{}, wave_pixel_block(P, t))) {
+#if RTC_TILE_DECODE
+            } else if (shade_ray<R, false>(sc, o, d, 0, sh, NoPush{}, wave_pixel_block(P, wt))) {
+#else
+            } else if (shade_ray<R, false>(sc, o, d, 0, sh, NoPush{}, wave_pixel_block(P, wave_tile(P, t)))) {
+#endif
 #elif RTC_AREA_LIGHTS
             } else if (shade_ray<R, false>(sc, o, d, P.max_depth, sh)) {
 #else
@@ -3058,6 +3161,19 @@
 #endif
 
 #if RTC_PRECISION != 2 && !RTC_INSTANCES
+__global__ void unit_vectors(const float* __restrict__ in, float* __restrict__ out, uint32_t n) {
+    const uint32_t i = threadIdx.x;
+    if (i >= n) return;
+    const V3<float> v = normalized(V3<float>{in[3 * i], in[3 * i + 1], in[3 * i + 2]});
+    out[3 * i] = v.x;
+    out[3 * i + 1] = v.y;
+    out[3 * i + 2] = v.z;
+}
+hipError_t launch_unit_vectors(const float* in, float* out, uint32_t n, hipStream_t stream) {
+    (void)hipGetLastError();
+    hipLaunchKernelGGL(unit_vectors, dim3(1), dim3(64), 0, stream, in, out, n);
+    return hipGetLastError();
+}
 hipError_t launch_canvas_signal(unsigned long long* flag, unsigned long long seq, hipStream_t stream) {
     (void)hipGetLastError();
     hipLaunchKernelGGL(canvas_signal, dim3(1), dim3(64), 0, stream, flag, seq);
```

Measured after the change: 475,500 Mray/s (median of 6 runs). 6.4% higher.
